# cszheng-ioa/Sixty-years-of-frequency-domain-monaural-speech-enhancement

Hardware: AMD Instinct MI355X
Metric: utterances/sec, 16 kHz 4 s clips, DCCRN decode (STFT->network->iSTFT) (higher is better)
Workload: dtype f32; 1 GPU; BASELINE configs[2]: DCCRN complex-mask, compressed input (0.5/2.0), 16 kHz x 4 s clips, batch 256 per MI355X, utterance-sharded; batch_per_gpu=256, global_batch=256, clip_samples=64000, parallelism=utterance shard x1 + RCCL gather to rank 0

## Files before the change

sixty-years-of-frequency-domain-monaural-speech-enhancement_amd/csrc/gemmconv.h:

```cpp
#pragma once
#include <hip/hip_runtime.h>
#include <vector>

namespace se {

constexpr int GC_MAX_TAPS = 16;
constexpr int GC_MAX_ROWS = 8;
constexpr int GC_MAX_KCP = 48;
constexpr int GC_TAB_KOFF = GC_MAX_ROWS + 2 * GC_MAX_TAPS;
constexpr int gc_kcp_max(int BM) { return 32; }
constexpr int gc_bld_max(int BM) { return (BM >= 128 || BM <= 32) ? 9 : 13; }
constexpr int gc_blocks_per_cu(int BM) { return BM <= 32 ? 6 : 3; }

enum Act : int { ACT_NONE = 0, ACT_PRELU = 1, ACT_ELU = 2, ACT_SOFTPLUS = 3, ACT_SIGMOID = 4, ACT_TANH = 5, ACT_RELU = 6 };
enum Epi : int {
    EPI_ACT = 0,
    EPI_LSTM = 1,
    EPI_GLU = 2,
    EPI_ADD = 3,
    EPI_MUL = 4,
    EPI_CMB = 5,
};

constexpr int GC_THIN_NT = 8;

struct GCParams {
    const float* A;
    const float* Ws;
    const float* bias;
    const float* slope;
    const float* post_scale;
    const float* post_shift;
    const float* bias_pad;
    int pad_lo;
    long ps_z;
    int cmb_neg;
    const float* cmb_i;
    float* cmb_s;
    const float* src0;
    const float* src1;
    float* dst;
    float* dst_elu;
    const float* aux;
    float* cell;
    long A_z, bias_z, src0_z, src1_z, dst_z, aux_z, cell_z;
    long s0_b, s0_c, s0_f;
    long s1_b, s1_c, s1_f;
    long d_b, d_c, d_f;
    long x_b, x_c, x_f;
    int C0, C1;
    int Fin, Tin;
    int B, Q, Tout, M, Mp;
    int si, so, po;
    int ntaps, nrows, dtmin, Wp;
    int CI_C, KC, KCp, nchunks;
    int act, epi;
    int n_ttiles, n_mtiles, Z;
    int dbg;
    int first_step;
    int gru;
    unsigned long long* timing;
    const unsigned* desc4;
    int t_base;
    int tb_soft;
    int pw4;
    int causal;
    const int* tlen;
    int qt2, qq_off, Qt;
    int pair, po2, fo_lim;
    short tdf[GC_MAX_TAPS], tdt[GC_MAX_TAPS];
    int nbuf;
    int trim;
    const unsigned* desc;
    const int* tab;
    float* stats;
    long st_b, st_c, st_f;
    float* cstats;
    long cs_b, cs_f;
    float* fz;
    long fz_b, fz_c, fz_f, fz_im;
    long fz_s;
    const float* nrm0;
    const float* nrm1;
    int flat_upr;
    int flat_units;
};
constexpr int GC_NRM_MAXC = 128;
constexpr int GC_FLAT_NRM_ROWS = 2;

struct GCGeom {
    int* tab = nullptr;
    unsigned* desc = nullptr;
    unsigned* desc4 = nullptr;
};
struct GCTail {
    int BN = 0, Wp = 0;
    GCGeom g;
};

struct GCSmallGeom {
    int dfmin = 0, dfmax = 0, dtmin = 0, dtmax = 0;
};

struct GCPlan {
    GCParams p{};
    int BM = 128, BN = 128;
    int lookback = 0;
    double flop_scale = 1.0;
    float* dA = nullptr;
    float* dWs = nullptr;
    unsigned* dDesc = nullptr;
    unsigned* dDesc4 = nullptr;
    GCSmallGeom small;
    bool tail_split = false;
    GCTail tail[3];
    GCTail qt2;
    GCTail flat[2];
    int flat_uw = 0;
    int qt2_nrows = 0, qt2_qoff = 0;
    float* dBias = nullptr;
    float* dSlope = nullptr;
    int* dTab = nullptr;
    float* dBiasPad = nullptr;
    float* dPostScale = nullptr;
    float* dPostShift = nullptr;
};

struct TapSpec {
    int ntaps = 0;
    int df[GC_MAX_TAPS];
    int dt[GC_MAX_TAPS];
};

GCPlan gc_make_plan(int M, int Cin, const TapSpec& taps, const std::vector<float>& w_logical,
                    const std::vector<float>& bias, const std::vector<float>& slope, int act, int epi,
                    int si, int so, int po, int tout_hint, int z = 1, int C0split = -1);
void gc_free_plan(GCPlan& pl);

void gc_register_overread_range(const void* lo, size_t bytes);
void gc_unregister_overread_range(const void* lo);

bool gc_stats_supported(const GCPlan& pl);
bool gc_nrm_supported(const GCPlan& pl);
void gc_launch(const GCPlan& pl, GCParams p, hipStream_t stream);
bool gc_launch_thin_pair(const GCParams& p0, const GCParams& p1, hipStream_t stream);

enum GCFamily : int { GC_FAM_TILE = 0, GC_FAM_THIN = 1, GC_FAM_THIN_PAIR = 2, GC_FAM_DIRECT = 3, GC_FAM_DIRECT_LDS = 4 };
struct GCLaunchRec {
    int family = GC_FAM_TILE;
    int BM = 0, BN = 0;
    int flat_upr = 0, upt = 0;
    int flat_rows = 0;
    int qt2 = 0, nrm = 0, res = 0, trim = 0, stats = 0, ragged = 0;
    int flat_nrm_refused = 0;
    long nblk = 0;
    int epi = 0, gru = 0;
};
void gc_set_launch_log(std::vector<GCLaunchRec>* log);
int gc_flat_rows_spanned(int B, int upr, int upt);

}
```

sixty-years-of-frequency-domain-monaural-speech-enhancement_amd/csrc/gemmconv.hip:

```cpp
#include "gemmconv.h"
#include "common.h"
#include "fastmath.h"
#include <algorithm>
#include <cmath>
#include <cstring>
#include <mutex>
#include <type_traits>

namespace se {

typedef float floatx16 __attribute__((ext_vector_type(16)));
typedef float floatx4 __attribute__((ext_vector_type(4)));

template <int N, typename F>
__device__ __forceinline__ void static_for(F&& f) {
    if constexpr (N > 0) {
        static_for<N - 1>(f);
        f(std::integral_constant<int, N - 1>{});
    }
}

__device__ __forceinline__ float fsig_(float x) { return fm_sigmoid(x); }
__device__ __forceinline__ float ftanh_(float x) { return fm_tanh(x); }
__device__ __forceinline__ float act_apply(float v, int act, float slope) {
    switch (act) {
        case ACT_PRELU: return v >= 0.f ? v : slope * v;
        case ACT_ELU: return v > 0.f ? v : fm_expm1(v);
        case ACT_SOFTPLUS: return fm_softplus(v);
        case ACT_SIGMOID: return fsig_(v);
        case ACT_TANH: return ftanh_(v);
        case ACT_RELU: return fmaxf(v, 0.f);
        default: return v;
    }
}
__device__ __forceinline__ float sigmoidf_(float v) { return 1.f / (1.f + expf(-v)); }
__device__ __forceinline__ float gc_fuse1(float v, float* __restrict__ zr, long im, long so = 0) {
    const float re = zr[0], ii = zr[im];
    const float cm = fm_sqrt(fmaxf(re * re + ii * ii, 1.1920928955078125e-07f));
    const float s = fsig_(v);
    zr[0] = re + s;
    zr[im] = ii + s;
    if (so) zr[so] = (re + s) + (ii + s);
    return v + fsig_(cm);
}

__device__ __forceinline__ void gc_dma16(const float* g, float* lds_wave_base) {
    const unsigned l = __builtin_amdgcn_readfirstlane((unsigned)(size_t)(__attribute__((address_space(3))) float*)lds_wave_base);
    asm volatile("s_mov_b32 m0, %0\n\ts_nop 0\n\tglobal_load_lds_dwordx4 %1, off" ::"s"(l), "v"(g) : "memory");
}
__device__ __forceinline__ void gc_dma4_masked(const float* g, unsigned lds_wave_base, unsigned pred) {
    unsigned long long saved;
    asm volatile(
        "s_mov_b64 %0, exec\n\t"
        "v_cmp_ne_u32_e32 vcc, 0, %1\n\t"
        "s_and_b64 exec, exec, vcc\n\t"
        "s_mov_b32 m0, %2\n\t"
        "s_nop 0\n\t"
        "global_load_lds_dword %3, off\n\t"
        "s_mov_b64 exec, %0"
        : "=&s"(saved)
        : "v"(pred), "s"(__builtin_amdgcn_readfirstlane(lds_wave_base)), "v"(g)
        : "memory", "vcc");
}
__device__ __forceinline__ void gc_dma16_masked(const float* g, unsigned lds_wave_base, unsigned pred) {
    unsigned long long saved;
    asm volatile(
        "s_mov_b64 %0, exec\n\t"
        "v_cmp_ne_u32_e32 vcc, 0, %1\n\t"
        "s_and_b64 exec, exec, vcc\n\t"
        "s_mov_b32 m0, %2\n\t"
        "s_nop 0\n\t"
        "global_load_lds_dwordx4 %3, off\n\t"
        "s_mov_b64 exec, %0"
        : "=&s"(saved)
        : "v"(pred), "s"(__builtin_amdgcn_readfirstlane(lds_wave_base)), "v"(g)
        : "memory", "vcc");
}
__device__ __forceinline__ void gc_dma16_s(const float* base, unsigned voff, unsigned lds_byte) {
    asm volatile("s_mov_b32 m0, %0\n\ts_nop 0\n\tglobal_load_lds_dwordx4 %1, %2" ::"s"(lds_byte), "v"(voff), "s"(base) : "memory");
}
__device__ __forceinline__ void gc_dma4_masked_s(const float* base, unsigned voff, unsigned lds_byte, unsigned vbits, unsigned mask) {
    unsigned long long saved;
    unsigned tmp;
    asm volatile(
        "s_mov_b64 %0, exec\n\t"
        "v_and_b32_e32 %1, %6, %2\n\t"
        "v_cmp_ne_u32_e32 vcc, 0, %1\n\t"
        "s_and_b64 exec, exec, vcc\n\t"
        "s_mov_b32 m0, %3\n\t"
        "s_nop 0\n\t"
        "global_load_lds_dword %4, %5\n\t"
        "s_mov_b64 exec, %0"
        : "=&s"(saved), "=&v"(tmp)
        : "v"(vbits), "s"(lds_byte), "v"(voff), "s"(base), "s"(mask)
        : "memory", "vcc");
}
__device__ __forceinline__ void gc_dma16_masked_s(const float* base, unsigned voff, unsigned lds_byte, unsigned vbits, unsigned mask) {
    unsigned long long saved;
    unsigned tmp;
    asm volatile(
        "s_mov_b64 %0, exec\n\t"
        "v_and_b32_e32 %1, %6, %2\n\t"
        "v_cmp_ne_u32_e32 vcc, 0, %1\n\t"
        "s_and_b64 exec, exec, vcc\n\t"
        "s_mov_b32 m0, %3\n\t"
        "s_nop 0\n\t"
        "global_load_lds_dwordx4 %4, %5\n\t"
        "s_mov_b64 exec, %0"
        : "=&s"(saved), "=&v"(tmp)
        : "v"(vbits), "s"(lds_byte), "v"(voff), "s"(base), "s"(mask)
        : "memory", "vcc");
}
__device__ __forceinline__ unsigned lds_addr(const float* p) {
    return (unsigned)(size_t)(__attribute__((address_space(3))) const float*)p;
}

#ifdef GC_TIMING
#define GC_T(SLOT)                                                               \
    {                                                                            \
        const unsigned long long now_ = __builtin_amdgcn_s_memtime();            \
        if (tid == 0) tacc[SLOT] += now_ - tlast;                                \
        tlast = __builtin_amdgcn_s_memtime();                                    \
    }
#else
#define GC_T(SLOT)
#endif

__device__ __forceinline__ float dpp_add8(float x) {
    x += __int_as_float(__builtin_amdgcn_update_dpp(0, __float_as_int(x), 0xB1, 0xF, 0xF, true));
    x += __int_as_float(__builtin_amdgcn_update_dpp(0, __float_as_int(x), 0x4E, 0xF, 0xF, true));
    x += __int_as_float(__builtin_amdgcn_update_dpp(0, __float_as_int(x), 0x141, 0xF, 0xF, true));
    return x;
}

template <int BM, int BN, int WM, int WN, int EPI, bool RES = false, bool TRIM = false, bool FZ = false, bool NRM = false, int FLATW = 0>
__global__ __launch_bounds__(256, RES ? 1 : (FZ || (BM >= 128 && BN >= 256)) ? (BM <= 32 ? 4 : 2) : gc_blocks_per_cu(BM)) void gc_kernel(const GCParams p) {
#ifdef GC_TIMING
    unsigned long long tacc[12] = {0, 0, 0, 0, 0, 0, 0, 0, 0, 0, 0, 0};
    unsigned long long tlast = __builtin_amdgcn_s_memtime();
#endif
    constexpr int TM = BM / (WM * 32);
    constexpr int TN = BN / (WN * 32);
    constexpr bool FLAT = FLATW > 0;
    constexpr int UW = FLAT ? FLATW : 32;
    constexpr int UPT = BN / 32;
    static_assert(!FLAT || (!RES && !TRIM && !FZ && EPI != EPI_LSTM), "flattened column tiles: plain offline variants only");
    constexpr int KCP_MAX = gc_kcp_max(BM);
    constexpr int A_IT = (KCP_MAX * BM / 4 + 255) / 256;
    constexpr int NB = BN >= 256 ? (BM >= 128 ? 6 : 5) : gc_bld_max(BM);
    static_assert(WM * WN == 4, "4 waves");

    extern __shared__ __attribute__((aligned(16))) float smem[];
    const int rows = p.CI_C * p.nrows;
    const int npatch = rows * p.Wp;
    const int bit = (npatch + 255) >> 8;
    const bool pw4 = p.pw4 != 0;
    constexpr bool fixt = TRIM;
    const int bit4 = (npatch / 4 + 255) >> 8;
    const int nA4 = p.KCp * (BM / 4);
    const int ait = (nA4 + 255) >> 8;
    const int As_sz = ait * 1024;
    const int Bs_sz = bit * 256;
    const int nbuf = RES ? p.nbuf : 2;
    float* As = smem;
    float* Bs = smem + nbuf * As_sz;

    const int tid = threadIdx.x;
    const int lane = tid & 63;
    const int wave = tid >> 6;
    const unsigned wave_u = __builtin_amdgcn_readfirstlane((unsigned)wave);
    const int l31 = lane & 31;
    const int hi = lane >> 5;

    int lid;
    {
        const int nblk = gridDim.x, id = blockIdx.x;
        const int xcd = id & 7, slot = id >> 3, q8 = nblk >> 3, r8 = nblk & 7;
        lid = (xcd < r8 ? xcd * (q8 + 1) : r8 * (q8 + 1) + (xcd - r8) * q8) + slot;
    }
    const int mt = lid % p.n_mtiles;
    int rest = lid / p.n_mtiles;
    const int ttile = FLAT ? (rest / p.Qt) % p.n_ttiles : rest % p.n_ttiles;
    if (FLAT) rest = (rest % p.Qt) + (rest / (p.Qt * p.n_ttiles)) * p.Qt;
    else rest /= p.n_ttiles;
    const bool qt2 = !FLAT && p.qt2 != 0;
    const int q = (rest % p.Qt) << (qt2 ? 1 : 0);
    rest /= p.Qt;
    const int u0 = FLAT ? ttile * UPT : 0;
    const int b = FLAT ? u0 / p.flat_upr : rest % p.B;
    const int z = FLAT ? rest : rest / p.B;
    const int t0 = FLAT ? p.t_base + (u0 - b * p.flat_upr) * 32 : p.t_base + ttile * (qt2 ? BN / 2 : BN);
    const int m0 = mt * BM;

    const float* __restrict__ Ag = p.A + (long)z * p.A_z + m0;

    constexpr int NPAIR = KCP_MAX / 2;
    constexpr bool KOFF_REGS = (BM >= 128 || TM * TN >= 4);
    int koffv[KOFF_REGS ? NPAIR : 1];
    constexpr int STRIPS = 4 * (TM * 32) * 36;
    int* tabl = reinterpret_cast<int*>(smem + max(nbuf * (As_sz + Bs_sz), STRIPS + (p.cstats ? 2048 : 0)));
    int* koff_lds = tabl + GC_TAB_KOFF;
    float* ep = reinterpret_cast<float*>(tabl + GC_TAB_KOFF + KCP_MAX + 8);
    constexpr int NRMB = FLAT ? GC_FLAT_NRM_ROWS : 1;
    static_assert(GC_FLAT_NRM_ROWS == 2, "the nrmC / nrmK fills below serve a tile's first row and the one after it");
    floatx4* nrmC = reinterpret_cast<floatx4*>(ep + 4 * BM);
    floatx4* nrmK = nrmC + NRMB * GC_NRM_MAXC;
    int* utab = reinterpret_cast<int*>(nrmC + (NRM ? NRMB * GC_NRM_MAXC + 2 * NRMB * KCP_MAX + 2 : 0));
    float* cpart = smem + STRIPS;
    GC_T(7);
    const int tabv = (tid < GC_TAB_KOFF + KCP_MAX + 8) ? p.tab[tid] : 0;
    const int fo = q * p.so + p.po;
    const float* __restrict__ bias = (fo < p.pad_lo) ? p.bias_pad : (p.bias ? p.bias + (long)z * p.bias_z : nullptr);
    float epv[4] = {0.f, 0.f, 1.f, 0.f};
    if (EPI != EPI_LSTM && tid < BM) {
        const int m = min(m0 + tid, p.M - 1);
        epv[0] = bias ? bias[m] : 0.f;
        const float lin_slope = p.act == ACT_NONE ? 1.f : 0.f;
        if (EPI == EPI_CMB) {
            epv[0] = p.post_shift[(long)z * p.ps_z + m];
            epv[1] = p.slope ? p.slope[(long)z * p.ps_z + m] : 1.f;
            epv[2] = p.post_scale[(long)z * p.ps_z + m];
        } else if (EPI != EPI_GLU) {
            epv[1] = (p.act == ACT_PRELU && p.slope) ? p.slope[m] : lin_slope;
        } else if (tid < BM / 2) {
            const int oc = min((m0 >> 1) + tid, (p.M >> 1) - 1);
            epv[1] = (p.act == ACT_PRELU && p.slope) ? p.slope[oc] : lin_slope;
            epv[2] = p.post_scale ? p.post_scale[oc] : 1.f;
            epv[3] = p.post_scale ? p.post_shift[oc] : 0.f;
        }
    }
    if constexpr (NRM) {
        const int ct_ = p.C0 + p.C1;
        if (tid < NRMB * ct_) {
            const int db_ = tid >= ct_ ? 1 : 0, ch_ = tid - db_ * ct_;
            const bool s1 = ch_ >= p.C0;
            const float* __restrict__ np_ = s1 ? p.nrm1 : p.nrm0;
            floatx4 v = {1.f, 0.f, 0.f, 0.f};
            if (np_) v = reinterpret_cast<const floatx4*>(np_)[(long)min(b + db_, p.B - 1) * (s1 ? p.C1 : p.C0) + (s1 ? ch_ - p.C0 : ch_)];
            nrmC[db_ * GC_NRM_MAXC + ch_] = v;
        }
    }
    if constexpr (FLAT) {
        if (tid < UPT) {
            const int u_ = u0 + tid, bk_ = u_ / p.flat_upr;
            utab[4 * tid + 0] = bk_ - b;
            utab[4 * tid + 1] = p.t_base + (u_ - bk_ * p.flat_upr) * 32;
            utab[4 * tid + 2] = u_ < p.flat_units ? 1 : 0;
            utab[4 * tid + 3] = p.tlen ? p.tlen[min(bk_, p.B - 1)] : 0x7fffffff;
        }
    }
    for (int i = tid; i < nbuf * Bs_sz / 4; i += 256) reinterpret_cast<floatx4*>(Bs)[i] = floatx4{0.f, 0.f, 0.f, 0.f};
    if (tid < GC_TAB_KOFF + KCP_MAX + 8) tabl[tid] = tabv;
    if (EPI != EPI_LSTM && tid < BM) {
        ep[tid] = epv[0];
        ep[BM + tid] = epv[1];
        if (EPI == EPI_GLU && tid < BM / 2) {
            ep[2 * BM + tid] = epv[2];
            ep[3 * BM + tid] = epv[3];
        }
        if (EPI == EPI_CMB) ep[2 * BM + tid] = epv[2];
    }
    __syncthreads();
    if constexpr (KOFF_REGS) {
        static_for<NPAIR>([&](auto KP) {
            constexpr int kp = decltype(KP)::value;
            koffv[kp] = koff_lds[2 * kp + hi];
        });
    }

    int nk_cil = 0, pb_cil = 0;
    bool nk_ok = false;
    const int npadL = (NRM && !FLAT) ? max(0, -(t0 + p.dtmin)) : 0;
    if constexpr (NRM) {
        if (tid < NRMB * KCP_MAX) {
            const int kr_ = tid & (KCP_MAX - 1);
            nk_cil = kr_ / p.ntaps;
            const int f = q * p.si + tabl[tabl[GC_MAX_ROWS + kr_ - nk_cil * p.ntaps]];
            nk_ok = kr_ < p.KC && f >= 0 && f < p.Fin;
        }
        pb_cil = tid / p.nrows;
    }

    unsigned aoff[A_IT];
    static_for<A_IT>([&](auto I) {
        constexpr int i = decltype(I)::value;
        int idx = tid + i * 256;
        if (idx >= nA4) idx = nA4 - 1;
        aoff[i] = 4u * (unsigned)((idx / (BM / 4)) * p.Mp + (idx % (BM / 4)) * 4);
    });
    unsigned boff[NB];
    unsigned vbits = 0;
    unsigned fullbits = 0;

    floatx16 acc[TM][TN];
#pragma unroll
    for (int i = 0; i < TM; ++i)
#pragma unroll
        for (int j = 0; j < TN; ++j)
#pragma unroll
            for (int r = 0; r < 16; ++r) acc[i][j][r] = 0.f;

    const int wm = wave / WN, wn = (WN == 4 && BN >= 256) ? ((wave + ttile) & 3) : wave % WN;
    constexpr int WNT = WN >= 2 ? WN / 2 : 1;
    const int wq = (qt2 && WN >= 2) ? wn / WNT : 0;
    const int wt = (qt2 && WN >= 2) ? wn % WNT : wn;
    const int am = wm * (TM * 32) + l31;
    const int bn = FLAT ? wn * (TN * UW) + l31 : wq * p.qq_off + wt * (TN * 32) + l31;
    const int jact = FLAT ? max(0, min(TN, p.flat_units - u0 - wn * TN))
                          : (q + wq >= p.Q) ? 0 : max(0, min(TN, (p.Tout - t0 - wt * (TN * 32) + 31) >> 5));

    int gchunk = 0;
    int buf = 0;

#define GC_MAKE_DESC(LIM)                                                                          \
    {                                                                                              \
        const int lim_ = (LIM);                                                                    \
        vbits = 0;                                                                                 \
         \
         \
         \
        unsigned dsc_[NB];                                                                         \
        {                                                                                          \
            const unsigned* __restrict__ dp_ = (pw4 ? p.desc4 : p.desc) + tid;                     \
            static_for<NB>([&](auto E) {                                                           \
                constexpr int e = decltype(E)::value;                                              \
                dsc_[e] = dp_[256 * e];                                                            \
            });                                                                                    \
        }                                                                                          \
        static_for<NB>([&](auto E) {                                                               \
            constexpr int e = decltype(E)::value;                                                  \
            const unsigned d_ = dsc_[e];                                                           \
            const int w = d_ & 0xfff, r = (d_ >> 12) & 0xf, cil = (d_ >> 16) & 0x7fff;             \
            const bool staged = (d_ >> 31) != 0;                                                   \
            const int f = q * p.si + tabl[staged ? r : 0];                                         \
             \
            const int uk_ = FLAT ? min(w / UW, UPT - 1) : 0;                                       \
            const int t = FLAT ? utab[4 * uk_ + 1] + p.dtmin + (w - uk_ * UW) : t0 + p.dtmin + w;  \
            const bool uok_ = !FLAT || utab[4 * uk_ + 2] != 0;                                     \
            const unsigned ub_ = (FLAT && uok_) ? (unsigned)utab[4 * uk_] * sb32 : 0u;             \
            const int fc = f < 0 ? 0 : (f >= p.Fin ? p.Fin - 1 : f);                               \
            const int tc = t < 0 ? 0 : (t >= p.Tin ? p.Tin - 1 : t);                               \
            const int cc = cil < lim_ ? cil : lim_ - 1;                                            \
            boff[e] = staged ? 4u * (ub_ + (unsigned)cc * sc32 + (unsigned)fc * sf32 + (unsigned)tc) : 0u;    \
             \
            vbits |= (staged && uok_ && (cil < lim_) && (f >= 0) && (f < p.Fin) && (t >= 0) && (t < p.Tin)) ? (1u << e) : 0u; \
             \
            if (fixt) vbits |= (staged && (t < p.Tin) && (t + 4 > p.Tin)) ? (0x10000u << e) : 0u;   \
        });                                                                                        \
         \
        fullbits = 0;       \
        {                                                                                          \
            if (!(p.dbg & 32)) static_for<NB>([&](auto E) {                                                           \
                constexpr int e = decltype(E)::value;                                              \
                if (e < bit4 && __builtin_amdgcn_ballot_w64((vbits >> e) & 1u) == ~0ull) fullbits |= 1u << e; \
            });                                                                                    \
        }                                                                                          \
    }
#define GC_TRIM_TAIL(BUF)                                                                          \
    if (fixt && (vbits >> 16)) {                                                                   \
        float* fb_ = Bs + (BUF) * Bs_sz + 4 * tid;                                                 \
        const int nv_ = p.Tin & 3;                                                                 \
        static_for<NB>([&](auto E) {                                                               \
            constexpr int e = decltype(E)::value;                                                  \
            if (vbits & (0x10000u << e)) {                                                         \
                _Pragma("unroll") for (int k = 1; k < 4; ++k)                                      \
                    if (k >= nv_) fb_[1024 * e + k] = 0.f;                                         \
            }                                                                                      \
        });                                                                                        \
    }
#define GC_LOAD_CHUNK(CH, BUF)                                                                     \
    {                                                                                              \
        if constexpr (NRM) {                                                                       \
             \
             \
            const int cb_ = (CH) * p.CI_C, co_ = seg ? p.C0 : 0;                                   \
            if (tid < NRMB * KCP_MAX) {                                                            \
                const int db_ = tid >= KCP_MAX ? 1 : 0;                                            \
                floatx4 v_ = nrmC[db_ * GC_NRM_MAXC + min(cb_ + nk_cil, Cseg - 1) + co_];          \
                if (!nk_ok) {                                                                      \
                    v_[0] = 0.f;                                                                   \
                    v_[1] = 0.f;                                                                   \
                }                                                                                  \
                nrmK[(BUF) * (NRMB * KCP_MAX) + tid] = v_;                                         \
            }                                                                                      \
            if (npadL > 0 && tid < rows) {                                                         \
                const float x0_ = nrmC[min(cb_ + pb_cil, Cseg - 1) + co_][3];                      \
                float* d_ = Bs + (BUF) * Bs_sz + tid * p.Wp;                                       \
                for (int w_ = 0; w_ < npadL; w_ += 4) *reinterpret_cast<floatx4*>(d_ + w_) = floatx4{x0_, x0_, x0_, x0_}; \
            }                                                                                      \
            if constexpr (FLAT) {       \
                if (tid < rows && p.dtmin < 0) {                                                   \
                    _Pragma("unroll") for (int k_ = 0; k_ < UPT; ++k_) {                           \
                        if (utab[4 * k_ + 1] + p.dtmin < 0 && utab[4 * k_ + 2]) {                  \
                            const float x0_ = nrmC[utab[4 * k_] * GC_NRM_MAXC + min(cb_ + pb_cil, Cseg - 1) + co_][3]; \
                            float* d_ = Bs + (BUF) * Bs_sz + tid * p.Wp + k_ * UW;                 \
                            for (int w_ = 0; w_ < -(utab[4 * k_ + 1] + p.dtmin); w_ += 4)          \
                                *reinterpret_cast<floatx4*>(d_ + w_) = floatx4{x0_, x0_, x0_, x0_}; \
                        }                                                                          \
                    }                                                                              \
                }                                                                                  \
            }                                                                                      \
        }                                                                                          \
         \
         \
        const float* __restrict__ Bc = sbase + (long)(CH) * p.CI_C * s_c;                          \
        const unsigned bb = __builtin_amdgcn_readfirstlane(lds_addr(Bs + (BUF) * Bs_sz));          \
        const unsigned bl = bb + 256u * wave_u, bl4 = bb + 1024u * wave_u;                         \
        if (pw4 && fullbits == (1u << bit4) - 1u) {      \
            static_for<NB>([&](auto E) {                                                           \
                constexpr int e = decltype(E)::value;                                              \
                if (e < bit4) gc_dma16_s(Bc, boff[e], bl4 + 4096u * e);                            \
            });                                                                                    \
        } else if (pw4) {                                                                          \
            static_for<NB>([&](auto E) {                                                           \
                constexpr int e = decltype(E)::value;                                              \
                if (e < bit4) gc_dma16_masked_s(Bc, boff[e], bl4 + 4096u * e, vbits, 1u << e);     \
            });                                                                                    \
        } else {                                                                                   \
            static_for<NB>([&](auto E) {                                                           \
                constexpr int e = decltype(E)::value;                                              \
                if (e < bit) gc_dma4_masked_s(Bc, boff[e], bl + 1024u * e, vbits, 1u << e);         \
            });                                                                                    \
        }                                                                                          \
        const float* __restrict__ Ac = Ag + (long)(gchunk + (CH)) * p.KCp * p.Mp;                  \
                                              \
        const unsigned Adw = __builtin_amdgcn_readfirstlane(lds_addr(As + (BUF) * As_sz)) + 1024u * wave_u; \
        static_for<A_IT>([&](auto I) {                                                             \
            constexpr int i = decltype(I)::value;                                                  \
            if (i < ait) gc_dma16_s(Ac, aoff[i], Adw + 4096u * i);                                 \
        });                                                                                        \
    }
#define GC_WAIT_CHUNK() asm volatile("s_waitcnt vmcnt(0)" ::: "memory")

    for (int seg = 0; seg < 2; ++seg) {
        const int Cseg = seg ? p.C1 : p.C0;
        if (Cseg <= 0) continue;
        const float* __restrict__ sbase =
            (seg ? p.src1 + (long)z * p.src1_z + (long)b * p.s1_b : p.src0 + (long)z * p.src0_z + (long)b * p.s0_b);
        const long s_c = seg ? p.s1_c : p.s0_c, s_f = seg ? p.s1_f : p.s0_f;
        const unsigned sc32 = (unsigned)s_c, sf32 = (unsigned)s_f;
        const unsigned sb32 = (unsigned)(seg ? p.s1_b : p.s0_b);
        const int nch = (Cseg + p.CI_C - 1) / p.CI_C;
        const int tail = Cseg - (nch - 1) * p.CI_C;

        GC_T(9);
        GC_MAKE_DESC(nch > 1 ? p.CI_C : tail);
        GC_T(10);
        if constexpr (RES) {
            buf = 0;
            for (int c2 = 0; c2 < min(nch, nbuf); ++c2) {
                if (c2 + 1 == nch && nch > 1 && tail != p.CI_C) GC_MAKE_DESC(tail);
                GC_LOAD_CHUNK(c2, c2);
            }
        } else {
            GC_LOAD_CHUNK(0, buf);
        }
        GC_T(1);
        GC_WAIT_CHUNK();
        GC_TRIM_TAIL(buf);
        GC_T(3);
        __syncthreads();
        GC_T(4);

        for (int c = 0; c < nch; ++c) {
            if constexpr (RES) {
                if (c > 0 && buf == nbuf) {
                    __syncthreads();
                    for (int c2 = c; c2 < min(nch, c + nbuf); ++c2) {
                        if (c2 + 1 == nch && tail != p.CI_C) GC_MAKE_DESC(tail);
                        GC_LOAD_CHUNK(c2, c2 - c);
                    }
                    GC_WAIT_CHUNK();
                    __syncthreads();
                    buf = 0;
                }
            }
            if (!RES && c + 1 < nch && !(p.dbg & 1)) {
                if (__builtin_expect(c + 2 == nch && tail != p.CI_C, 0)) GC_MAKE_DESC(tail);
                GC_LOAD_CHUNK(c + 1, buf ^ 1);
            }
            GC_T(1);
            const float* Ab = As + buf * As_sz + hi * BM + am;
            const float* Bb = Bs + buf * Bs_sz + bn;
            const floatx4* nkb = nrmK + buf * (NRMB * KCP_MAX) + hi;
            int nkd[FLAT && NRM ? TN : 1];
            if constexpr (FLAT && NRM) {
#pragma unroll
                for (int j = 0; j < TN; ++j) nkd[j] = utab[4 * min(wn * TN + j, UPT - 1)] * KCP_MAX;
            }
            const int npair = p.KCp >> 1;
#define GC_FETCH(KP, AR, BR)                                                                       \
    {                                                                                              \
        int o_;                                                                                    \
        if constexpr (KOFF_REGS) o_ = koffv[(KP) < NPAIR ? (KP) : NPAIR - 1];                      \
        else o_ = koff_lds[2 * (KP) + hi];                                                         \
        _Pragma("unroll") for (int i = 0; i < TM; ++i) AR[i] = Ab[(2 * (KP)) * BM + i * 32];       \
        _Pragma("unroll") for (int j = 0; j < JN; ++j) BR[j] = Bb[o_ + j * UW];                    \
        if constexpr (NRM && !FLAT) {                                                              \
            const floatx4 pr_ = nkb[2 * (KP)];                                                     \
            _Pragma("unroll") for (int j = 0; j < JN; ++j) {                                       \
                const float t_ = fmaf(BR[j], pr_[0], pr_[1]);                                      \
                BR[j] = fmaf(fminf(t_, 0.f), pr_[2], t_);                                          \
            }                                                                                      \
        }                                                                                          \
        if constexpr (NRM && FLAT) {                                                               \
            _Pragma("unroll") for (int j = 0; j < JN; ++j) {                                       \
                const floatx4 pr_ = nkb[2 * (KP) + nkd[j]];                                        \
                const float t_ = fmaf(BR[j], pr_[0], pr_[1]);                                      \
                BR[j] = fmaf(fminf(t_, 0.f), pr_[2], t_);                                          \
            }                                                                                      \
        }                                                                                          \
    }
#define GC_MMA(AR, BR)                                                                             \
    _Pragma("unroll") for (int i = 0; i < TM; ++i)                                                 \
        _Pragma("unroll") for (int j = 0; j < JN; ++j)                                             \
            acc[i][j] = __builtin_amdgcn_mfma_f32_32x32x2f32(AR[i], BR[j], acc[i][j], 0, 0, 0);
            auto mma_chunk = [&](auto JN_) {
                constexpr int JN = decltype(JN_)::value;
                float ax[TM], bx[JN], ay[TM], by[JN];
                GC_FETCH(0, ax, bx);
                static_for<NPAIR / 2>([&](auto KP2) {
                    constexpr int kp = 2 * decltype(KP2)::value;
                    int np_ = npair;
                    asm volatile("" : "+s"(np_));
                    if (kp < np_) {
                        constexpr int NDS = (TM + 1) / 2 + (JN + 1) / 2 + (NRM ? (FLAT ? JN : 1) : 0);
                        GC_FETCH(kp + 1, ay, by);
                        __builtin_amdgcn_sched_group_barrier(0x100, NDS, 0);
                        GC_MMA(ax, bx);
                        __builtin_amdgcn_sched_group_barrier(0x008, TM * JN, 0);
                        if constexpr (NRM) __builtin_amdgcn_sched_group_barrier(0x002, 3 * JN, 0);
                        GC_FETCH(kp + 2, ax, bx);
                        __builtin_amdgcn_sched_group_barrier(0x100, NDS, 0);
                        GC_MMA(ay, by);
                        __builtin_amdgcn_sched_group_barrier(0x008, TM * JN, 0);
                        if constexpr (NRM) __builtin_amdgcn_sched_group_barrier(0x002, 3 * JN, 0);
                    }
                });
            };
            if (!(p.dbg & 4)) {
                if (jact == 1 && TN == 2) mma_chunk(std::integral_constant<int, 1>{});
                else if (jact >= 1) mma_chunk(std::integral_constant<int, TN>{});
            }
#undef GC_FETCH
#undef GC_MMA
            GC_T(2);
            if constexpr (RES) {
                buf += 1;
            } else {
                GC_WAIT_CHUNK();
                GC_TRIM_TAIL(buf ^ 1);
                GC_T(3);
                __syncthreads();
                GC_T(4);
                buf ^= 1;
            }
        }
        if constexpr (RES) __syncthreads();
        gchunk += nch;
    }
#undef GC_MAKE_DESC
#undef GC_LOAD_CHUNK
#undef GC_WAIT_CHUNK
#undef GC_TRIM_TAIL

    if (p.dbg & 8) return;
    GC_T(0);
    const int fow = fo + wq * p.so;
    float* __restrict__ dst = p.dst + (long)z * p.dst_z + (long)b * p.d_b + (long)fow * p.d_f;

    constexpr int OROWS = (EPI == EPI_GLU) ? TM * 16 : TM * 32;
    constexpr bool GC_STATS = (EPI == EPI_GLU) || (EPI == EPI_ACT && BM == 64);
    constexpr int OST = 32 + 4;
    float* strip = smem + wave * (TM * 32 * OST);
#define GC_WAVE_FENCE() asm volatile("s_waitcnt lgkmcnt(0)" ::: "memory")
    if (EPI == EPI_ACT || EPI == EPI_ADD || EPI == EPI_MUL || EPI == EPI_GLU || EPI == EPI_CMB) {
        const int mw = wm * (TM * 32) + 4 * hi;
        const int lr = lane >> 3, lc = (lane & 7) * 4;
        const int mo0 = (EPI == EPI_GLU ? (m0 >> 1) : m0) + wm * OROWS;
        const int Mo = (q + wq < p.Q) ? ((EPI == EPI_GLU) ? (p.M >> 1) : p.M) : 0;
        const int tvalid0 = p.tlen ? p.tlen[b] : 0x7fffffff;
        const float* __restrict__ res =
            (EPI == EPI_ADD || EPI == EPI_MUL || EPI == EPI_CMB) ? p.aux + (long)z * p.aux_z + (long)b * p.x_b + (long)fow * p.x_f : nullptr;
        const float cmb_sg = (EPI == EPI_CMB && ((p.cmb_neg >> z) & 1)) ? -1.f : 1.f;
        const float* __restrict__ cmbi = (EPI == EPI_CMB && p.cmb_s) ? p.cmb_i + (long)b * p.d_b + (long)fow * p.d_f : nullptr;
        float* __restrict__ cmbs = (EPI == EPI_CMB && p.cmb_s) ? p.cmb_s + (long)b * p.d_b + (long)fow * p.d_f : nullptr;
        float* __restrict__ delu = (EPI == EPI_GLU && p.dst_elu) ? p.dst_elu + (long)b * p.d_b + (long)fow * p.d_f : nullptr;
        float* __restrict__ fzb = FZ ? p.fz + (long)b * p.fz_b + (long)fow * p.fz_f : nullptr;
        auto epi_tile = [&](auto jc) __attribute__((always_inline)) {
            constexpr int j = decltype(jc)::value;
            if (j > 0) GC_WAVE_FENCE();
            const int uk = FLAT ? min(wn * TN + j, UPT - 1) : 0;
            const long dbJ = FLAT ? utab[4 * uk] : 0;
            const int tj0 = FLAT ? utab[4 * uk + 1] : t0 + wt * (TN * 32) + j * 32;
            const int MoJ = (!FLAT || utab[4 * uk + 2]) ? Mo : 0;
            const int tvalid = FLAT ? utab[4 * uk + 3] : tvalid0;
            const int tstat = min(p.Tout, tvalid);
            float* __restrict__ dstJ = dst + dbJ * p.d_b;
            const float* __restrict__ resJ = res ? res + dbJ * p.x_b : nullptr;
            const float* __restrict__ cmbiJ = cmbi ? cmbi + dbJ * p.d_b : nullptr;
            float* __restrict__ cmbsJ = cmbs ? cmbs + dbJ * p.d_b : nullptr;
            float* __restrict__ deluJ = delu ? delu + dbJ * p.d_b : nullptr;
            constexpr bool PRE = (EPI == EPI_ADD || EPI == EPI_MUL || EPI == EPI_CMB);
            const int tgp = tj0 + lc;
            floatx4 rvp[PRE ? OROWS / 8 : 1], zre[FZ ? OROWS / 8 : 1], zim[FZ ? OROWS / 8 : 1], ivp[EPI == EPI_CMB ? OROWS / 8 : 1];
            if ((PRE || FZ) && tgp + 3 < p.Tout && MoJ > 0) {
#pragma unroll
                for (int it = 0; it < OROWS / 8; ++it) {
                    const int m = min(mo0 + it * 8 + lr, MoJ - 1);
                    if (PRE) rvp[it] = *reinterpret_cast<const floatx4*>(resJ + (long)m * p.x_c + tgp);
                    if (EPI == EPI_CMB && cmbiJ) ivp[it] = *reinterpret_cast<const floatx4*>(cmbiJ + (long)m * p.d_c + tgp);
                    if (FZ) {
                        zre[it] = *reinterpret_cast<const floatx4*>(fzb + (long)m * p.fz_c + tgp);
                        zim[it] = *reinterpret_cast<const floatx4*>(fzb + (long)m * p.fz_c + tgp + p.fz_im);
                    }
                }
            }
            auto write_strip = [&](auto ACT_) __attribute__((always_inline)) {
                constexpr int ACT = decltype(ACT_)::value;
                auto actf = [&](float v, float sl) __attribute__((always_inline)) -> float {
                    if constexpr (ACT == -2) return v;
                    else if constexpr (ACT < 0) return v >= 0.f ? v : sl * v;
                    else return act_apply(v, ACT, sl);
                };
                typedef float floatx2 __attribute__((ext_vector_type(2)));
#pragma unroll
                for (int i = 0; i < TM; ++i) {
                    if (EPI == EPI_CMB) {
#pragma unroll
                        for (int r = 0; r < 16; ++r) {
                            const int dm = i * 32 + (r & 3) + 8 * (r >> 2);
                            strip[(4 * hi + dm) * OST + l31] = acc[i][j][r];
                        }
                    } else if (EPI != EPI_GLU) {
#pragma unroll
                        for (int g4 = 0; g4 < 4; ++g4) {
                            const int dm0 = i * 32 + 8 * g4;
                            const floatx4 b4 = *reinterpret_cast<const floatx4*>(ep + mw + dm0);
                            floatx4 s4 = {1.f, 1.f, 1.f, 1.f};
                            if constexpr (ACT != -2) s4 = *reinterpret_cast<const floatx4*>(ep + BM + mw + dm0);
#pragma unroll
                            for (int k = 0; k < 4; ++k) {
                                const float v = acc[i][j][4 * g4 + k] + b4[k];
                                strip[(4 * hi + dm0 + k) * OST + l31] = actf(v, s4[k]);
                            }
                        }
                    } else {
#pragma unroll
                        for (int g4 = 0; g4 < 4; ++g4) {
                            const int dm0 = i * 32 + 8 * g4;
                            const int ol0 = (mw + dm0) >> 1;
                            const floatx4 b4 = *reinterpret_cast<const floatx4*>(ep + mw + dm0);
                            const floatx2 sc2 = *reinterpret_cast<const floatx2*>(ep + 2 * BM + ol0);
                            const floatx2 sh2 = *reinterpret_cast<const floatx2*>(ep + 3 * BM + ol0);
                            floatx2 sl2 = {1.f, 1.f};
                            if constexpr (ACT != -2) sl2 = *reinterpret_cast<const floatx2*>(ep + BM + ol0);
#pragma unroll
                            for (int k = 0; k < 2; ++k) {
                                const float a = acc[i][j][4 * g4 + 2 * k] + b4[2 * k];
                                const float g = acc[i][j][4 * g4 + 2 * k + 1] + b4[2 * k + 1];
                                float v = a * fsig_(g);
                                v = v * sc2[k] + sh2[k];
                                strip[(((4 * hi + dm0) >> 1) + k) * OST + l31] = actf(v, sl2[k]);
                            }
                        }
                    }
                }
            };
            switch (p.act) {
                case ACT_NONE: write_strip(std::integral_constant<int, -2>{}); break;
                case ACT_RELU:
                case ACT_PRELU: write_strip(std::integral_constant<int, -1>{}); break;
                case ACT_ELU: write_strip(std::integral_constant<int, ACT_ELU>{}); break;
                case ACT_SOFTPLUS: write_strip(std::integral_constant<int, ACT_SOFTPLUS>{}); break;
                case ACT_SIGMOID: write_strip(std::integral_constant<int, ACT_SIGMOID>{}); break;
                default: write_strip(std::integral_constant<int, ACT_TANH>{}); break;
            }
            GC_WAVE_FENCE();
            const int tg = tj0 + lc;
            constexpr int RB_UNROLL = (PRE || FZ) ? OROWS / 8 : 1;
            float ccs[GC_STATS ? 4 : 1] = {}, ccq[GC_STATS ? 4 : 1] = {};
            long doff = (long)(mo0 + lr) * p.d_c + tg;
            const long dstep = 8L * p.d_c;
            long soff = 0;
            if constexpr (GC_STATS) soff = (long)(b + dbJ) * p.st_b + (long)(mo0 + lr) * p.st_c + (long)fow * p.st_f + (tj0 >> 5) * 2;
            const long sstep = GC_STATS ? 8L * p.st_c : 0;
#pragma unroll RB_UNROLL
            for (int it = 0; it < OROWS / 8; ++it, doff += dstep, soff += sstep) {
                const int row = it * 8 + lr, m = mo0 + row;
                floatx4 v = *reinterpret_cast<const floatx4*>(strip + row * OST + lc);
                if constexpr (GC_STATS) {
                    if (p.cstats && m < MoJ) {
#pragma unroll
                        for (int k = 0; k < 4; ++k) {
                            const float xk = (tg + k < tstat) ? v[k] : 0.f;
                            ccs[k] += xk;
                            ccq[k] = fmaf(xk, xk, ccq[k]);
                        }
                    }
                }
                if constexpr (GC_STATS) {
                    if (p.stats) {
                        float s = 0.f, q = 0.f;
#pragma unroll
                        for (int k = 0; k < 4; ++k) {
                            const float xk = (tg + k < tstat) ? v[k] : 0.f;
                            s += xk;
                            q = fmaf(xk, xk, q);
                        }
                        s = dpp_add8(s);
                        q = dpp_add8(q);
                        const int tb = tg - lc;
                        if ((lane & 7) == 0 && m < MoJ && tb < p.Tout) {
                            float* sp = p.stats + soff;
                            sp[0] = s;
                            sp[1] = q;
                        }
                    }
                }
                if (m < MoJ) {
                    float* __restrict__ dp = dstJ + doff;
                    if (__builtin_expect(tg + 3 < p.Tout, 1)) {
                        if (EPI == EPI_ADD || EPI == EPI_MUL) v = (EPI == EPI_ADD) ? v + rvp[it] : v * rvp[it];
                        if (EPI == EPI_CMB) {
                            const int rt = wm * (TM * 32) + row;
                            const float sh_ = ep[rt], sl_ = ep[BM + rt], sc_ = ep[2 * BM + rt];
#pragma unroll
                            for (int k = 0; k < 4; ++k) {
                                const float u = fmaf(fmaf(cmb_sg, v[k], rvp[it][k]), sc_, sh_);
                                v[k] = u >= 0.f ? u : sl_ * u;
                            }
                        }
                        if (__builtin_expect(tg + 3 >= tvalid, 0)) {
#pragma unroll
                            for (int k = 0; k < 4; ++k) v[k] = (tg + k < tvalid) ? v[k] : 0.f;
                        }
                        if (FZ) {
                            float* __restrict__ zr = fzb + (long)m * p.fz_c + tg;
                            floatx4 re = zre[it], ii = zim[it];
#pragma unroll
                            for (int k = 0; k < 4; ++k) {
                                const float cm = fm_sqrt(fmaxf(re[k] * re[k] + ii[k] * ii[k], 1.1920928955078125e-07f));
                                const float sg = fsig_(v[k]);
                                re[k] += sg;
                                ii[k] += sg;
                                v[k] += fsig_(cm);
                            }
                            *reinterpret_cast<floatx4*>(zr) = re;
                            *reinterpret_cast<floatx4*>(zr + p.fz_im) = ii;
                            if (p.fz_s) *reinterpret_cast<floatx4*>(zr + p.fz_s) = re + ii;
                        }
                        *reinterpret_cast<floatx4*>(dp) = v;
                        if (EPI == EPI_GLU && deluJ) {
                            floatx4 e4;
#pragma unroll
                            for (int k = 0; k < 4; ++k) e4[k] = v[k] > 0.f ? v[k] : fm_expm1(v[k]);
                            *reinterpret_cast<floatx4*>(deluJ + doff) = e4;
                        }
                        if (EPI == EPI_CMB && cmbsJ) {
                            floatx4 s4 = v + ivp[it];
                            if (__builtin_expect(tg + 3 >= tvalid, 0)) {
#pragma unroll
                                for (int k = 0; k < 4; ++k) s4[k] = (tg + k < tvalid) ? s4[k] : 0.f;
                            }
                            *reinterpret_cast<floatx4*>(cmbsJ + doff) = s4;
                        }
                    } else {
#pragma unroll
                        for (int k = 0; k < 4; ++k)
                            if (tg + k < p.Tout) {
                                float o = v[k];
                                if (EPI == EPI_ADD) o += resJ[(long)m * p.x_c + tg + k];
                                if (EPI == EPI_MUL) o *= resJ[(long)m * p.x_c + tg + k];
                                if (EPI == EPI_CMB) {
                                    const int rt = wm * (TM * 32) + row;
                                    const float u = fmaf(fmaf(cmb_sg, o, resJ[(long)m * p.x_c + tg + k]), ep[2 * BM + rt], ep[rt]);
                                    o = u >= 0.f ? u : ep[BM + rt] * u;
                                }
                                o = (tg + k < tvalid) ? o : 0.f;
                                if (FZ) o = gc_fuse1(o, fzb + (long)m * p.fz_c + tg + k, p.fz_im, p.fz_s);
                                dp[k] = o;
                                if (EPI == EPI_GLU && deluJ) deluJ[doff + k] = o > 0.f ? o : fm_expm1(o);
                                if (EPI == EPI_CMB && cmbsJ) {
                                    const float iv = cmbiJ[doff + k];
                                    cmbsJ[doff + k] = (tg + k < tvalid) ? o + iv : 0.f;
                                }
                            }
                    }
                }
            }
            if constexpr (GC_STATS) {
                if (p.cstats) {
#pragma unroll
                    for (int k = 0; k < 4; ++k) {
                        ccs[k] += __int_as_float(__builtin_amdgcn_update_dpp(0, __float_as_int(ccs[k]), 0x128, 0xF, 0xF, true));
                        ccq[k] += __int_as_float(__builtin_amdgcn_update_dpp(0, __float_as_int(ccq[k]), 0x128, 0xF, 0xF, true));
                    }
                    if (!(lane & 8)) {
                        float* cp_ = cpart + (((wm * 4 + (lane >> 4)) * BN) + wt * (TN * 32) + j * 32 + lc) * 2;
#pragma unroll
                        for (int k = 0; k < 4; ++k) {
                            cp_[2 * k] = ccs[k];
                            cp_[2 * k + 1] = ccq[k];
                        }
                    }
                }
            }
        };
        epi_tile(std::integral_constant<int, 0>{});
        if constexpr (TN > 1) epi_tile(std::integral_constant<int, 1>{});
        if constexpr (TN > 2) {
            epi_tile(std::integral_constant<int, 2>{});
            epi_tile(std::integral_constant<int, 3>{});
        }
        static_assert(TN == 1 || TN == 2 || TN == 4, "epilogue: column tiles per wave");
        if constexpr (GC_STATS) {
            if (p.cstats) {
                __syncthreads();
                for (int col = tid; col < BN; col += 256) {
                    float a = 0.f, c2 = 0.f;
#pragma unroll
                    for (int w = 0; w < 4 * WM; ++w) {
                        a += cpart[(w * BN + col) * 2];
                        c2 += cpart[(w * BN + col) * 2 + 1];
                    }
                    const int ukc = FLAT ? col >> 5 : 0;
                    const int t = FLAT ? utab[4 * ukc + 1] + (col & 31) : t0 + col;
                    const long bc = FLAT ? b + utab[4 * ukc] : b;
                    if (t < p.Tout && fo < p.so * p.Q + p.po && (!FLAT || utab[4 * ukc + 2])) {
                        float* cg = p.cstats + bc * p.cs_b + (long)fo * p.cs_f + 2 * t;
                        cg[0] = a;
                        cg[1] = c2;
                    }
                }
            }
        }
    } else {
        const bool has_gx = p.aux != nullptr;
        const float* __restrict__ gx = has_gx ? p.aux + (long)z * p.aux_z + (long)b * p.x_b + (long)fo * p.x_f : p.bias;
        float* __restrict__ cell = p.cell + (long)z * p.cell_z + (long)b * p.d_b + (long)fo * p.d_f;
        float cpa[TM][TN][4];
#pragma unroll
        for (int i = 0; i < TM; ++i)
#pragma unroll
            for (int j = 0; j < TN; ++j) {
                const int tc = min(t0 + wn * (TN * 32) + j * 32 + l31, p.Tout - 1);
                const int mb = m0 + wm * (TM * 32) + i * 32 + 4 * hi;
#pragma unroll
                for (int g4 = 0; g4 < 4; ++g4) {
                    const int m = min(mb + 8 * g4, p.M - 4);
                    cpa[i][j][g4] = p.first_step ? 0.f : cell[(long)(m >> 2) * p.d_c + tc];
                }
            }
        auto cells = [&](auto GRU_, auto HGX_) __attribute__((always_inline)) {
            constexpr bool GRU = decltype(GRU_)::value, HGX = decltype(HGX_)::value;
#pragma unroll
        for (int i = 0; i < TM; ++i)
#pragma unroll
            for (int j = 0; j < TN; ++j) {
                const int t = t0 + wn * (TN * 32) + j * 32 + l31;
                const int tc = min(t, p.Tout - 1);
                const int mb = m0 + wm * (TM * 32) + i * 32 + 4 * hi;
                float g[16], cp[4];
#pragma unroll
                for (int g4 = 0; g4 < 4; ++g4) {
                    const int m = min(mb + 8 * g4, p.M - 4);
                    const float* gp = HGX ? gx + (long)m * p.x_c + tc : gx + m;
                    const long gs = HGX ? p.x_c : 1;
#pragma unroll
                    for (int k = 0; k < 4; ++k) g[4 * g4 + k] = gp[(long)k * gs];
                    cp[g4] = cpa[i][j][g4];
                }
#pragma unroll
                for (int g4 = 0; g4 < 4; ++g4) {
                    const int m = mb + 8 * g4;
                    const float gi = acc[i][j][4 * g4 + 0] + g[4 * g4 + 0];
                    const float gf = acc[i][j][4 * g4 + 1] + g[4 * g4 + 1];
                    const float gg = acc[i][j][4 * g4 + 2] + g[4 * g4 + 2];
                    const float go = acc[i][j][4 * g4 + 3] + g[4 * g4 + 3];
                    float cn, hn;
                    if constexpr (GRU) {
                        const float r = fsig_(gi), zz = fsig_(gf);
                        const float hw = acc[i][j][4 * g4 + 2] + go;
                        const float nn = ftanh_(g[4 * g4 + 2] + r * hw);
                        hn = (1.f - zz) * nn + zz * cp[g4];
                        cn = hn;
                    } else {
                        cn = fsig_(gf) * cp[g4] + fsig_(gi) * ftanh_(gg);
                        hn = fsig_(go) * ftanh_(cn);
                    }
                    if (m + 3 < p.M && t < p.Tout) {
                        const long oi = (long)(m >> 2) * p.d_c + t;
                        cell[oi] = cn;
                        dst[oi] = hn;
                    }
                }
            }
    
        };
        if (p.gru) {
            if (has_gx) cells(std::true_type{}, std::true_type{});
            else cells(std::true_type{}, std::false_type{});
        } else {
            if (has_gx) cells(std::false_type{}, std::true_type{});
            else cells(std::false_type{}, std::false_type{});
        }
    }
#ifdef GC_TIMING
    GC_T(5);
    if (tid == 0) {
        for (int i = 0; i < 6; ++i) atomicAdd(p.timing + i, tacc[i]);
        for (int i = 7; i < 12; ++i) atomicAdd(p.timing + i, tacc[i]);
        atomicAdd(p.timing + 6, 1ull);
    }
#endif
}

template <int MM, int EPI>
__global__ __launch_bounds__(256) void gc_small_kernel(const GCParams p) {
    __shared__ int s_df[GC_MAX_TAPS], s_dt[GC_MAX_TAPS];
    if (threadIdx.x < p.ntaps) {
        s_df[threadIdx.x] = p.tab[p.tab[GC_MAX_ROWS + threadIdx.x]];
        s_dt[threadIdx.x] = p.tab[GC_MAX_ROWS + GC_MAX_TAPS + threadIdx.x];
    }
    __syncthreads();
    int lid;
    {
        const int nblk = gridDim.x, id = blockIdx.x;
        const int xcd = id & 7, slot = id >> 3, q8 = nblk >> 3, r8 = nblk & 7;
        lid = (xcd < r8 ? xcd * (q8 + 1) : r8 * (q8 + 1) + (xcd - r8) * q8) + slot;
    }
    const int q = lid % p.Q;
    int rest = lid / p.Q;
    const int nt = (p.Tout + 255) >> 8;
    const int tt = rest % nt;
    rest /= nt;
    const int b = rest % p.B, z = rest / p.B;
    const int t = tt * 256 + threadIdx.x;
    const int tc = min(t, p.Tout - 1);
    float acc[MM];
#pragma unroll
    for (int m = 0; m < MM; ++m) acc[m] = 0.f;
    const float* __restrict__ W = p.Ws + (long)z * (p.C0 + p.C1) * p.ntaps * MM;
#pragma unroll 1
    for (int seg = 0; seg < 2; ++seg) {
        const int C = seg ? p.C1 : p.C0;
        if (C == 0) continue;
        const float* __restrict__ src = seg ? p.src1 + (long)z * p.src1_z + (long)b * p.s1_b
                                            : p.src0 + (long)z * p.src0_z + (long)b * p.s0_b;
        const long s_c = seg ? p.s1_c : p.s0_c, s_f = seg ? p.s1_f : p.s0_f;
        const float* __restrict__ Wc = W + (long)(seg ? p.C0 : 0) * p.ntaps * MM;
        for (int j = 0; j < p.ntaps; ++j) {
            const int fi = q * p.si + s_df[j], ti = tc + s_dt[j];
            const bool ok = fi >= 0 && fi < p.Fin && ti >= 0 && ti < p.Tin;
            const float* __restrict__ xp = src + (long)min(max(fi, 0), p.Fin - 1) * s_f + min(max(ti, 0), p.Tin - 1);
            const float keep = ok ? 1.f : 0.f;
#pragma unroll 8
            for (int c = 0; c < C; ++c) {
                const float x = xp[(long)c * s_c] * keep;
                const float* __restrict__ w = Wc + ((long)c * p.ntaps + j) * MM;
#pragma unroll
                for (int m = 0; m < MM; ++m) acc[m] = fmaf(w[m], x, acc[m]);
            }
        }
    }
    if (t >= p.Tout) return;
    const int fo = q * p.so + p.po;
    const float* __restrict__ bias = (fo < p.pad_lo) ? p.bias_pad : (p.bias ? p.bias + (long)z * p.bias_z : nullptr);
    float* __restrict__ dst = p.dst + (long)z * p.dst_z + (long)b * p.d_b + (long)fo * p.d_f;
    const float* __restrict__ res = (EPI == EPI_ADD || EPI == EPI_MUL) ? p.aux + (long)z * p.aux_z + (long)b * p.x_b + (long)fo * p.x_f : nullptr;
    if constexpr (EPI == EPI_GLU) {
#pragma unroll
        for (int j = 0; j < MM / 2; ++j) {
            if (2 * j + 1 < p.M) {
                const float a = acc[2 * j] + (bias ? bias[2 * j] : 0.f), g = acc[2 * j + 1] + (bias ? bias[2 * j + 1] : 0.f);
                float v = a * fsig_(g);
                if (p.post_scale) v = v * p.post_scale[j] + p.post_shift[j];
                v = act_apply(v, p.act, p.slope ? p.slope[j] : 0.f);
                if (p.pair) {
                    const int cls = (2 * j) / p.pair, fo2 = q * p.so + (cls ? p.po2 : p.po);
                    if (fo2 < p.fo_lim) dst[(long)(fo2 - fo) * p.d_f + (long)(j - cls * (p.pair >> 1)) * p.d_c + t] = v;
                } else {
                    dst[(long)j * p.d_c + t] = v;
                }
            }
        }
        return;
    }
#pragma unroll
    for (int m = 0; m < MM; ++m) {
        if (m < p.M) {
            float v = acc[m] + (bias ? bias[m] : 0.f);
            v = act_apply(v, p.act, p.slope ? p.slope[m] : 0.f);
            if (EPI == EPI_ADD) v += res[(long)m * p.x_c + t];
            if (EPI == EPI_MUL) v *= res[(long)m * p.x_c + t];
            if (EPI == EPI_ACT && p.pair) {
                const int cls = m / p.pair, fo2 = q * p.so + (cls ? p.po2 : p.po);
                if (fo2 < p.fo_lim) dst[(long)(fo2 - fo) * p.d_f + (long)(m - cls * p.pair) * p.d_c + t] = v;
                continue;
            }
            dst[(long)m * p.d_c + t] = v;
        }
    }
}

constexpr int SQB = 8;
constexpr int SWT = 264;
template <int MM, int EPI, int SI>
__global__ __launch_bounds__(256) void gc_small_lds_kernel(const GCParams p, const int CC, const int NR, const int dfmin,
                                                           const int dtlo) {
    extern __shared__ float patch[];
    __shared__ int s_off[GC_MAX_TAPS];
    __shared__ float s_w[8 * GC_MAX_TAPS * MM];
    const int tid = threadIdx.x, lane = tid & 63, wave = tid >> 6;
    if (tid < p.ntaps)
        s_off[tid] = (p.tab[p.tab[GC_MAX_ROWS + tid]] - dfmin) * SWT + (p.tab[GC_MAX_ROWS + GC_MAX_TAPS + tid] - dtlo);
    const int QG = (p.Q + SQB - 1) / SQB;
    int rest = blockIdx.x;
    const int q0 = (rest % QG) * SQB;
    rest /= QG;
    const int nt = (p.Tout + 255) >> 8;
    const int tt = rest % nt;
    rest /= nt;
    const int b = rest % p.B, z = rest / p.B;
    const int t = tt * 256 + tid;
    const int f0 = q0 * SI + dfmin, tb = tt * 256 + dtlo;
    float acc[SQB][MM];
#pragma unroll
    for (int qq = 0; qq < SQB; ++qq)
#pragma unroll
        for (int m = 0; m < MM; ++m) acc[qq][m] = 0.f;
    const float* __restrict__ W = p.Ws + (long)z * (p.C0 + p.C1) * p.ntaps * MM;
    const int plane = NR * SWT;
#pragma unroll 1
    for (int seg = 0; seg < 2; ++seg) {
        const int C = seg ? p.C1 : p.C0;
        if (C == 0) continue;
        const float* __restrict__ src = seg ? p.src1 + (long)z * p.src1_z + (long)b * p.s1_b
                                            : p.src0 + (long)z * p.src0_z + (long)b * p.s0_b;
        const long s_c = seg ? p.s1_c : p.s0_c, s_f = seg ? p.s1_f : p.s0_f;
        const float* __restrict__ Wc = W + (long)(seg ? p.C0 : 0) * p.ntaps * MM;
        constexpr int SRB = 6, SWN = (SWT + 63) / 64, SWW = (8 * GC_MAX_TAPS * MM + 255) / 256;
        float sv[SRB][SWN], wv[SWW];
        auto issue = [&](int c0n) {
            const int ccn = min(CC, C - c0n);
#pragma unroll
            for (int i = 0; i < SRB; ++i) {
                const int row = min(wave + 4 * i, ccn * NR - 1);
                const int c = row / NR, r = row - c * NR;
                const float* __restrict__ sp = src + (long)(c0n + c) * s_c + (long)min(max(f0 + r, 0), p.Fin - 1) * s_f;
#pragma unroll
                for (int k = 0; k < SWN; ++k) sv[i][k] = sp[min(max(tb + lane + 64 * k, 0), p.Tin - 1)];
            }
#pragma unroll
            for (int k = 0; k < SWW; ++k) wv[k] = Wc[(long)c0n * p.ntaps * MM + min(tid + 256 * k, ccn * p.ntaps * MM - 1)];
        };
        issue(0);
#pragma unroll 1
        for (int c0 = 0; c0 < C; c0 += CC) {
            const int cc = min(CC, C - c0);
            __syncthreads();
#pragma unroll
            for (int k = 0; k < SWW; ++k)
                if (tid + 256 * k < cc * p.ntaps * MM) s_w[tid + 256 * k] = wv[k];
#pragma unroll
            for (int i = 0; i < SRB; ++i) {
                const int row = wave + 4 * i;
                if (row < cc * NR) {
                    const int c = row / NR, r = row - c * NR;
                    const int fi = f0 + r;
                    const bool rok = fi >= 0 && fi < p.Fin;
                    float* __restrict__ dp = patch + c * plane + r * SWT;
#pragma unroll
                    for (int k = 0; k < SWN; ++k) {
                        const int w = lane + 64 * k, ti = tb + w;
                        if (w < SWT) dp[w] = (rok && ti >= 0 && ti < p.Tin) ? sv[i][k] : 0.f;
                    }
                }
            }
            if (c0 + CC < C) issue(c0 + CC);
            __syncthreads();
            for (int c = 0; c < cc; ++c) {
                const float* __restrict__ pc = patch + c * plane + tid;
                const float* wc = s_w + c * p.ntaps * MM;
#pragma unroll 2
                for (int j = 0; j < p.ntaps; ++j) {
                    const float* __restrict__ pj = pc + s_off[j];
                    float w[MM];
#pragma unroll
                    for (int m = 0; m < MM; ++m) w[m] = wc[j * MM + m];
#pragma unroll
                    for (int qq = 0; qq < SQB; ++qq) {
                        const float x = pj[qq * SI * SWT];
#pragma unroll
                        for (int m = 0; m < MM; ++m) acc[qq][m] = fmaf(w[m], x, acc[qq][m]);
                    }
                }
            }
        }
    }
    if (t >= p.Tout) return;
#pragma unroll
    for (int qq = 0; qq < SQB; ++qq) {
        if (q0 + qq >= p.Q) break;
        const int fo = (q0 + qq) * p.so + p.po;
        const float* __restrict__ bias = (fo < p.pad_lo) ? p.bias_pad : (p.bias ? p.bias + (long)z * p.bias_z : nullptr);
        float* __restrict__ dst = p.dst + (long)z * p.dst_z + (long)b * p.d_b + (long)fo * p.d_f;
        const float* __restrict__ res = (EPI == EPI_ADD || EPI == EPI_MUL) ? p.aux + (long)z * p.aux_z + (long)b * p.x_b + (long)fo * p.x_f : nullptr;
        if constexpr (EPI == EPI_GLU) {
#pragma unroll
            for (int j = 0; j < MM / 2; ++j) {
                if (2 * j + 1 < p.M) {
                    const float a = acc[qq][2 * j] + (bias ? bias[2 * j] : 0.f), g = acc[qq][2 * j + 1] + (bias ? bias[2 * j + 1] : 0.f);
                    float v = a * fsig_(g);
                    if (p.post_scale) v = v * p.post_scale[j] + p.post_shift[j];
                    v = act_apply(v, p.act, p.slope ? p.slope[j] : 0.f);
                    if (p.pair) {
                        const int cls = (2 * j) / p.pair, fo2 = (q0 + qq) * p.so + (cls ? p.po2 : p.po);
                        if (fo2 < p.fo_lim) dst[(long)(fo2 - fo) * p.d_f + (long)(j - cls * (p.pair >> 1)) * p.d_c + t] = v;
                    } else {
                        dst[(long)j * p.d_c + t] = v;
                    }
                }
            }
            continue;
        }
#pragma unroll
        for (int m = 0; m < MM; ++m) {
            if (m < p.M) {
                float v = acc[qq][m] + (bias ? bias[m] : 0.f);
                v = act_apply(v, p.act, p.slope ? p.slope[m] : 0.f);
                if (EPI == EPI_ADD) v += res[(long)m * p.x_c + t];
                if (EPI == EPI_MUL) v *= res[(long)m * p.x_c + t];
                if (EPI == EPI_ACT && p.pair) {
                    const int cls = m / p.pair, fo2 = (q0 + qq) * p.so + (cls ? p.po2 : p.po);
                    if (fo2 < p.fo_lim) dst[(long)(fo2 - fo) * p.d_f + (long)(m - cls * p.pair) * p.d_c + t] = v;
                    continue;
                }
                dst[(long)m * p.d_c + t] = v;
            }
        }
    }
}

template <int EPI, int NT>
__device__ __forceinline__ void gc_thin_body(const GCParams& p, const int blk) {
    constexpr int RB = 8, KG = 32, UN = 8;
    __shared__ float part[KG][RB][NT + 1];
    __shared__ int s_df[GC_MAX_TAPS], s_dt[GC_MAX_TAPS];
    const int tid = threadIdx.x, mi = tid & (RB - 1), kg = tid / RB;
#pragma unroll
    for (int j = 0; j < GC_MAX_TAPS; ++j)
        if (tid == j) {
            s_df[j] = p.tdf[j];
            s_dt[j] = p.tdt[j];
        }
    __syncthreads();
    const int nm = (p.M + RB - 1) / RB;
    const int mt = blk % nm;
    const int rest = blk / nm;
    const int q = rest % p.Q, b = rest / p.Q;
    const int m = mt * RB + mi, t0 = p.t_base, n = p.Tout - p.t_base;
    const int ntaps = p.ntaps, Ktot = (p.C0 + p.C1) * ntaps;
    const int nch0 = p.C0 > 0 ? (p.C0 + p.CI_C - 1) / p.CI_C : 0;
    float acc[NT];
#pragma unroll
    for (int t = 0; t < NT; ++t) acc[t] = 0.f;
    for (int k0 = kg; k0 < Ktot; k0 += KG * UN) {
        float w[UN], xv[UN][NT];
#pragma unroll
        for (int u = 0; u < UN; ++u) {
            const int kk = k0 + u * KG;
            const bool kok = kk < Ktot;
            const int kc = kok ? kk : 0;
            const int ci = kc / ntaps, j = kc - ci * ntaps;
            const bool seg = ci >= p.C0;
            const int cs = seg ? ci - p.C0 : ci;
            const int chunk = (seg ? nch0 : 0) + cs / p.CI_C, cil = cs % p.CI_C;
            const float wv = p.A[((long)chunk * p.KCp + cil * ntaps + j) * p.Mp + m];
            const int f = q * p.si + s_df[j];
            const bool fok = kok && f >= 0 && f < p.Fin;
            const int fc = fok ? f : 0;
            const float* __restrict__ src = seg ? p.src1 + (long)b * p.s1_b + (long)cs * p.s1_c + (long)fc * p.s1_f
                                                : p.src0 + (long)b * p.s0_b + (long)cs * p.s0_c + (long)fc * p.s0_f;
            const int tb = t0 + s_dt[j];
            w[u] = fok ? wv : 0.f;
#pragma unroll
            for (int t = 0; t < NT; ++t) {
                const int ti = tb + t;
                const bool ok = t < n && ti >= 0 && ti < p.Tin;
                const float x = src[ok ? ti : 0];
                xv[u][t] = ok ? x : 0.f;
            }
        }
#pragma unroll
        for (int u = 0; u < UN; ++u)
#pragma unroll
            for (int t = 0; t < NT; ++t) acc[t] = fmaf(w[u], xv[u][t], acc[t]);
    }
#pragma unroll
    for (int t = 0; t < NT; ++t) part[kg][mi][t] = acc[t];
    __syncthreads();
    const bool fold = tid < RB * NT;
    const int r = tid & (RB - 1), t = (tid / RB) & (NT - 1);
    float tot = 0.f;
    if (fold) {
#pragma unroll
        for (int g = 0; g < KG; ++g) tot += part[g][r][t];
    }
    __syncthreads();
    if (fold) part[0][r][t] = tot;
    __syncthreads();
    if (!fold || t >= n) return;
    const int fo = q * p.so + p.po, mr = mt * RB + r;
    const float* __restrict__ bias = (fo < p.pad_lo) ? p.bias_pad : p.bias;
    float* __restrict__ dst = p.dst + (long)b * p.d_b + (long)fo * p.d_f + t0 + t;
    if (EPI == EPI_LSTM) {
        if ((r & 3) || mr + 3 >= p.M) return;
        const int tc = t0 + t;
        const bool has_gx = p.aux != nullptr;
        const float* __restrict__ gx = has_gx ? p.aux + (long)b * p.x_b + (long)fo * p.x_f + (long)mr * p.x_c + tc : p.bias + mr;
        const long gs = has_gx ? p.x_c : 1;
        float* __restrict__ cell = p.cell + (long)b * p.d_b + (long)fo * p.d_f + (long)(mr >> 2) * p.d_c + tc;
        const float g0 = gx[0], g1 = gx[gs], g2 = gx[2 * gs], g3 = gx[3 * gs];
        const float cp = p.first_step ? 0.f : *cell;
        const float gi = part[0][r][t] + g0, gf = part[0][r + 1][t] + g1, gg = part[0][r + 2][t] + g2, go = part[0][r + 3][t] + g3;
        float cn, hn;
        if (p.gru) {
            const float rr = fsig_(gi), zz = fsig_(gf);
            const float hw = part[0][r + 2][t] + go;
            const float nn = ftanh_(g2 + rr * hw);
            hn = (1.f - zz) * nn + zz * cp;
            cn = hn;
        } else {
            cn = fsig_(gf) * cp + fsig_(gi) * ftanh_(gg);
            hn = fsig_(go) * ftanh_(cn);
        }
        *cell = cn;
        dst[(long)(mr >> 2) * p.d_c] = hn;
    } else if (EPI == EPI_GLU) {
        if ((r & 1) || mr + 1 >= p.M) return;
        const int oc = mr >> 1;
        const float a = part[0][r][t] + (bias ? bias[mr] : 0.f), g = part[0][r + 1][t] + (bias ? bias[mr + 1] : 0.f);
        float v = a * fsig_(g);
        if (p.post_scale) v = v * p.post_scale[oc] + p.post_shift[oc];
        dst[(long)oc * p.d_c] = act_apply(v, p.act, p.slope ? p.slope[oc] : 0.f);
    } else {
        if (mr >= p.M) return;
        float v = part[0][r][t] + (bias ? bias[mr] : 0.f);
        v = act_apply(v, p.act, p.slope ? p.slope[mr] : 0.f);
        if (EPI == EPI_ADD || EPI == EPI_MUL) {
            const float rv = p.aux[(long)b * p.x_b + (long)fo * p.x_f + (long)mr * p.x_c + t0 + t];
            v = (EPI == EPI_ADD) ? v + rv : v * rv;
        }
        dst[(long)mr * p.d_c] = v;
    }
}
template <int EPI, int NT>
__global__ __launch_bounds__(256) void gc_thin_kernel(const GCParams p) {
    gc_thin_body<EPI, NT>(p, (int)blockIdx.x);
}
struct GCThinPair {
    GCParams p[2];
    int nblk0;
};
template <int EPI, int NT>
__global__ __launch_bounds__(256) void gc_thin_pair_kernel(const GCThinPair a) {
    const int cls = (int)blockIdx.x >= a.nblk0 ? 1 : 0;
    gc_thin_body<EPI, NT>(a.p[cls], (int)blockIdx.x - (cls ? a.nblk0 : 0));
}
template <int EPI>
static void gc_thin_launch_n(const GCParams& p, dim3 grid, int n, hipStream_t stream) {
    if (n <= 1) hipLaunchKernelGGL((gc_thin_kernel<EPI, 1>), grid, dim3(256), 0, stream, p);
    else if (n <= 2) hipLaunchKernelGGL((gc_thin_kernel<EPI, 2>), grid, dim3(256), 0, stream, p);
    else if (n <= 4) hipLaunchKernelGGL((gc_thin_kernel<EPI, 4>), grid, dim3(256), 0, stream, p);
    else hipLaunchKernelGGL((gc_thin_kernel<EPI, 8>), grid, dim3(256), 0, stream, p);
}
static thread_local std::vector<GCLaunchRec>* g_launch_log = nullptr;
static thread_local int g_flat_nrm_refused = 0;
void gc_set_launch_log(std::vector<GCLaunchRec>* log) { g_launch_log = log; }
static void gc_log_launch(int family, const GCParams& p, long nblk, int BM = 0, int BN = 0, bool res = false) {
    if (!g_launch_log) return;
    GCLaunchRec r;
    r.family = family;
    r.BM = BM;
    r.BN = BN;
    r.flat_upr = p.flat_upr;
    r.upt = p.flat_upr ? BN / 32 : 0;
    r.flat_rows = p.flat_upr ? gc_flat_rows_spanned(p.B, p.flat_upr, BN / 32) : 0;
    r.qt2 = p.qt2;
    r.nrm = (p.nrm0 || p.nrm1) ? 1 : 0;
    r.res = res ? 1 : 0;
    r.trim = p.trim;
    r.stats = (p.stats || p.cstats) ? 1 : 0;
    r.ragged = p.tlen ? 1 : 0;
    r.flat_nrm_refused = g_flat_nrm_refused;
    r.nblk = nblk;
    r.epi = p.epi;
    r.gru = p.gru;
    g_launch_log->push_back(r);
}
int gc_flat_rows_spanned(int B, int upr, int upt) {
    const long units = (long)B * upr, tiles = (units + upt - 1) / upt;
    int most = 0;
    for (long k = 0; k < std::min<long>(tiles, upr); ++k) {
        const long u0 = k * upt, u1 = std::min(u0 + upt, units) - 1;
        most = std::max(most, (int)(u1 / upr - u0 / upr + 1));
    }
    return most;
}

constexpr long GC_THIN_MAX_BLOCKS = 8192;
static long gc_thin_blocks(const GCParams& p) {
    const int n = p.Tout - p.t_base;
    if ((p.Ws && p.pair) || n > GC_THIN_NT || p.Z > 1 || p.stats || p.cstats || p.nrm0 || p.nrm1) return 0;
    if (p.epi != EPI_ACT && p.epi != EPI_ADD && p.epi != EPI_MUL && p.epi != EPI_GLU && p.epi != EPI_LSTM) return 0;
    if (p.epi == EPI_LSTM && (p.M & 3)) return 0;
    const long nblk = (long)((p.M + 7) >> 3) * p.Q * p.B;
    if (nblk > GC_THIN_MAX_BLOCKS) return 0;
    if (!p.Ws) {
        const int nt = n <= 1 ? 1 : (n <= 2 ? 2 : (n <= 4 ? 4 : 8));
        const double waves_thin = std::ceil((double)nblk / 2048.0);
        const double waves_mfma = std::ceil((double)std::max(p.Z, 1) * p.B * p.Q * std::max(p.n_mtiles, 1) / 512.0);
        if ((long)p.B * n > 64 || nblk > 2800 * waves_mfma || waves_thin * (1 + nt) > 12 * waves_mfma) return 0;
    }
    return nblk;
}
static bool gc_thin_launch(const GCParams& p, hipStream_t stream) {
    const long nblk = (p.fz || p.dst_elu) ? 0 : gc_thin_blocks(p);
    if (nblk <= 0) return false;
    const int n = p.Tout - p.t_base;
    dim3 grid((unsigned)nblk);
    switch (p.epi) {
        case EPI_ACT: gc_thin_launch_n<EPI_ACT>(p, grid, n, stream); break;
        case EPI_ADD: gc_thin_launch_n<EPI_ADD>(p, grid, n, stream); break;
        case EPI_MUL: gc_thin_launch_n<EPI_MUL>(p, grid, n, stream); break;
        case EPI_GLU: gc_thin_launch_n<EPI_GLU>(p, grid, n, stream); break;
        case EPI_LSTM: gc_thin_launch_n<EPI_LSTM>(p, grid, n, stream); break;
        default: return false;
    }
    SE_HIP(hipGetLastError());
    gc_log_launch(GC_FAM_THIN, p, nblk);
    return true;
}

template <int EPI>
static void gc_thin_pair_launch_n(const GCThinPair& a, dim3 grid, int n, hipStream_t stream) {
    if (n <= 1) hipLaunchKernelGGL((gc_thin_pair_kernel<EPI, 1>), grid, dim3(256), 0, stream, a);
    else if (n <= 2) hipLaunchKernelGGL((gc_thin_pair_kernel<EPI, 2>), grid, dim3(256), 0, stream, a);
    else if (n <= 4) hipLaunchKernelGGL((gc_thin_pair_kernel<EPI, 4>), grid, dim3(256), 0, stream, a);
    else hipLaunchKernelGGL((gc_thin_pair_kernel<EPI, 8>), grid, dim3(256), 0, stream, a);
}
bool gc_launch_thin_pair(const GCParams& p0, const GCParams& p1, hipStream_t stream) {
    const long n0 = gc_thin_blocks(p0), n1 = gc_thin_blocks(p1);
    if (n0 <= 0 || n1 <= 0 || p0.epi != p1.epi || p0.Tout - p0.t_base != p1.Tout - p1.t_base) return false;
    GCThinPair a;
    a.p[0] = p0;
    a.p[1] = p1;
    a.nblk0 = (int)n0;
    const int n = p0.Tout - p0.t_base;
    dim3 grid((unsigned)(n0 + n1));
    switch (p0.epi) {
        case EPI_ACT: gc_thin_pair_launch_n<EPI_ACT>(a, grid, n, stream); break;
        case EPI_ADD: gc_thin_pair_launch_n<EPI_ADD>(a, grid, n, stream); break;
        case EPI_MUL: gc_thin_pair_launch_n<EPI_MUL>(a, grid, n, stream); break;
        case EPI_GLU: gc_thin_pair_launch_n<EPI_GLU>(a, grid, n, stream); break;
        default: return false;
    }
    SE_HIP(hipGetLastError());
    gc_log_launch(GC_FAM_THIN_PAIR, p0, n0 + n1);
    return true;
}

template <int MM, int EPI>
static void gc_small_lds_launch(const GCParams& p, dim3 grid, size_t shm, int CC, int NR, const GCSmallGeom& sg, hipStream_t stream) {
    if (p.si == 1) hipLaunchKernelGGL((gc_small_lds_kernel<MM, EPI, 1>), grid, dim3(256), shm, stream, p, CC, NR, sg.dfmin, sg.dtmin);
    else hipLaunchKernelGGL((gc_small_lds_kernel<MM, EPI, 2>), grid, dim3(256), shm, stream, p, CC, NR, sg.dfmin, sg.dtmin);
}

template <int MM>
static void gc_small_launch(const GCParams& p, const GCSmallGeom& sg, hipStream_t stream) {
    const int NR = (SQB - 1) * p.si + (sg.dfmax - sg.dfmin) + 1;
    constexpr int small_kb = 24;
    const int CC = std::min(std::min(8, 24 / std::max(NR, 1)), (int)((size_t)small_kb * 1024 / ((size_t)NR * SWT * sizeof(float))));
    const long nblk8 = (long)((p.Tout + 255) / 256) * ((p.Q + SQB - 1) / SQB) * p.B * p.Z;
    if (CC >= 2 && p.Q >= SQB && (p.si == 1 || p.si == 2) && sg.dtmax - sg.dtmin <= SWT - 256 && nblk8 >= 4 * 256 &&
        (sg.dfmax - sg.dfmin >= 2 || (sg.dfmax - sg.dfmin >= 1 && MM >= 2 && p.C0 + p.C1 >= 64))) {
        SE_CHECK(nblk8 < (1L << 31), "grid size");
        const size_t shm = (size_t)CC * NR * SWT * sizeof(float);
        dim3 grid((unsigned)nblk8);
        switch (p.epi) {
            case EPI_ACT: gc_small_lds_launch<MM, EPI_ACT>(p, grid, shm, CC, NR, sg, stream); break;
            case EPI_ADD: gc_small_lds_launch<MM, EPI_ADD>(p, grid, shm, CC, NR, sg, stream); break;
            case EPI_MUL: gc_small_lds_launch<MM, EPI_MUL>(p, grid, shm, CC, NR, sg, stream); break;
            case EPI_GLU:
                if constexpr (MM >= 2) gc_small_lds_launch<MM, EPI_GLU>(p, grid, shm, CC, NR, sg, stream);
                break;
            default: SE_CHECK(false, "direct small-M path: unsupported epilogue");
        }
        SE_HIP(hipGetLastError());
        gc_log_launch(GC_FAM_DIRECT_LDS, p, nblk8);
        return;
    }
    const long nblk = (long)((p.Tout + 255) / 256) * p.Q * p.B * p.Z;
    SE_CHECK(nblk > 0 && nblk < (1L << 31), "grid size");
    dim3 grid((unsigned)nblk);
    switch (p.epi) {
        case EPI_ACT: hipLaunchKernelGGL((gc_small_kernel<MM, EPI_ACT>), grid, dim3(256), 0, stream, p); break;
        case EPI_ADD: hipLaunchKernelGGL((gc_small_kernel<MM, EPI_ADD>), grid, dim3(256), 0, stream, p); break;
        case EPI_MUL: hipLaunchKernelGGL((gc_small_kernel<MM, EPI_MUL>), grid, dim3(256), 0, stream, p); break;
        case EPI_GLU:
            if constexpr (MM >= 2) hipLaunchKernelGGL((gc_small_kernel<MM, EPI_GLU>), grid, dim3(256), 0, stream, p);
            break;
        default: SE_CHECK(false, "direct small-M path: unsupported epilogue");
    }
    SE_HIP(hipGetLastError());
    gc_log_launch(GC_FAM_DIRECT, p, nblk);
}

static size_t gc_lds_bytes(const GCParams& p, int BM, size_t epi_bytes, int nbuf = 2) {
    const size_t as = (size_t)((p.KCp * (BM / 4) + 255) / 256) * 1024, bs = (size_t)((p.CI_C * p.nrows * p.Wp + 255) / 256) * 256;
    const size_t nrb = p.flat_upr ? GC_FLAT_NRM_ROWS : 1;
    const size_t nrm = ((p.nrm0 || p.nrm1) ? (size_t)(nrb * GC_NRM_MAXC + 2 * nrb * gc_kcp_max(BM) + 2) * 16 : 0) + (p.flat_upr ? 128 : 0);
    const size_t cst = p.cstats ? (size_t)4 * 256 * 2 * 4 : 0;
    return std::max((size_t)nbuf * (as + bs) * 4, epi_bytes + cst) + (GC_TAB_KOFF + GC_MAX_KCP + 8) * 4 + (size_t)4 * BM * 4 + 64 + nrm;
}

GCGeom gc_build_geom(const TapSpec& taps, const std::vector<int>& rows, int dtmin, int nrows, int Wp, int cic, int KC, int NB) {
    GCGeom g;
    std::vector<int> tab(GC_TAB_KOFF + GC_MAX_KCP + 8, 0);
    for (int r = 0; r < nrows; ++r) tab[r] = rows[r];
    for (int j = 0; j < taps.ntaps; ++j) {
        tab[GC_MAX_ROWS + j] = (int)(std::find(rows.begin(), rows.end(), taps.df[j]) - rows.begin());
        tab[GC_MAX_ROWS + GC_MAX_TAPS + j] = taps.dt[j];
    }
    for (int k = 0; k < KC; ++k) {
        const int cil = k / taps.ntaps, j = k - cil * taps.ntaps;
        tab[GC_TAB_KOFF + k] = cil * (nrows * Wp) + tab[GC_MAX_ROWS + j] * Wp + (taps.dt[j] - dtmin);
    }
    SE_HIP(hipMalloc(&g.tab, tab.size() * sizeof(int)));
    SE_HIP(hipMemcpy(g.tab, tab.data(), tab.size() * sizeof(int), hipMemcpyHostToDevice));
    const int npatch = cic * nrows * Wp, gpr = Wp / 4;
    SE_CHECK(Wp % 4 == 0 && Wp < 4096 && nrows <= 16 && cic < 32768, "patch descriptor field overflow");
    std::vector<unsigned> desc((size_t)NB * 256, 0u), d4((size_t)NB * 256, 0u);
    for (int e = 0; e < NB; ++e)
        for (int t = 0; t < 256; ++t) {
            const int fe = t + 256 * e;
            if (fe < npatch) {
                const int rr = fe / Wp, w = fe - rr * Wp, cil = rr / nrows, r = rr - cil * nrows;
                desc[(size_t)e * 256 + t] = (unsigned)w | ((unsigned)r << 12) | ((unsigned)cil << 16) | 0x80000000u;
            }
            if (4 * fe < npatch) {
                const int rr = fe / gpr, w = 4 * (fe - rr * gpr), cil = rr / nrows, r = rr - cil * nrows;
                d4[(size_t)e * 256 + t] = (unsigned)w | ((unsigned)r << 12) | ((unsigned)cil << 16) | 0x80000000u;
            }
        }
    SE_HIP(hipMalloc(&g.desc, desc.size() * sizeof(unsigned)));
    SE_HIP(hipMemcpy(g.desc, desc.data(), desc.size() * sizeof(unsigned), hipMemcpyHostToDevice));
    SE_HIP(hipMalloc(&g.desc4, d4.size() * sizeof(unsigned)));
    SE_HIP(hipMemcpy(g.desc4, d4.data(), d4.size() * sizeof(unsigned), hipMemcpyHostToDevice));
    return g;
}

GCPlan gc_make_plan(int M, int Cin, const TapSpec& taps, const std::vector<float>& w, const std::vector<float>& bias,
                    const std::vector<float>& slope, int act, int epi, int si, int so, int po, int tout_hint, int Z,
                    int C0split) {
    const int C0 = (C0split < 0 || C0split > Cin) ? Cin : C0split;
    SE_CHECK(taps.ntaps >= 1 && taps.ntaps <= GC_MAX_TAPS, "tap count");
    SE_CHECK((long)w.size() == (long)Z * M * Cin * taps.ntaps, "weight size mismatch in gc_make_plan");
    GCPlan pl;
    GCParams& p = pl.p;
    pl.BM = M >= 96 ? 128 : (M >= 48 ? 64 : 32);
    {
        static const int pw64 = getenv("SE_GC_PW_BM64") ? atoi(getenv("SE_GC_PW_BM64")) : 128;
        if (pw64 > 0 && taps.ntaps == 1 && Cin <= pw64 && M >= 96 && M <= 384 && epi != EPI_LSTM) pl.BM = 64;
    }
    pl.BN = (tout_hint >= 96 || pl.BM == 32) ? 128 : 64;
    int dtmin = taps.dt[0], dtmax = taps.dt[0];
    std::vector<int> rows;
    for (int j = 0; j < taps.ntaps; ++j) {
        dtmin = std::min(dtmin, taps.dt[j]);
        dtmax = std::max(dtmax, taps.dt[j]);
        if (std::find(rows.begin(), rows.end(), taps.df[j]) == rows.end()) rows.push_back(taps.df[j]);
    }
    std::sort(rows.begin(), rows.end());
    SE_CHECK((int)rows.size() <= GC_MAX_ROWS, "too many distinct frequency rows");
    p.ntaps = taps.ntaps;
    p.nrows = (int)rows.size();
    for (int j = 0; j < taps.ntaps; ++j) {
        SE_CHECK(taps.df[j] >= -32768 && taps.df[j] <= 32767 && taps.dt[j] >= -32768 && taps.dt[j] <= 32767, "tap offset range");
        p.tdf[j] = (short)taps.df[j];
        p.tdt[j] = (short)taps.dt[j];
    }
    p.causal = dtmax <= 0;
    pl.lookback = std::max(-dtmin, 0);
    dtmin = -((std::max(-dtmin, 0) + 3) & ~3);
    dtmax = (std::max(dtmax, 0) + 3) & ~3;
    p.dtmin = dtmin;
    p.Wp = pl.BN + (dtmax - dtmin);
    SE_CHECK(p.nrows * p.Wp <= gc_bld_max(pl.BM) * 256, "tap span too wide for one staged patch");
    int cic = 1;
    double best = -1.0;
    for (int c = 1; c <= std::max(std::max(C0, Cin - C0), 1); ++c) {
        const int kc = c * taps.ntaps, kcp = (kc + 3) & ~3;
        const bool pw = taps.ntaps == 1;
        const int kmax = pw ? (pl.BM >= 128 ? 24 : 32) : gc_kcp_max(pl.BM);
        const int cap = gc_bld_max(pl.BM) * 256 * (pw ? 4 : 1);
        if (kcp > kmax || c * p.nrows * p.Wp > cap) continue;
        if (pl.BM == 64 && pl.BN == 128 && taps.ntaps > 1 && epi != EPI_LSTM && kc > 12 &&
            (long)c * p.nrows * (256 + (dtmax - dtmin)) > 4608)
            continue;
        const double score = (double)kc / kcp + 1e-4 * kc;
        if (score > best) {
            best = score;
            cic = c;
        }
    }
    p.CI_C = cic;
    p.KC = cic * taps.ntaps;
    p.KCp = (p.KC + 3) & ~3;
    SE_CHECK(p.KCp <= gc_kcp_max(pl.BM), "single-channel chunk exceeds K budget");
    {
        GCGeom g = gc_build_geom(taps, rows, dtmin, p.nrows, p.Wp, cic, p.KC, gc_bld_max(pl.BM));
        pl.dTab = g.tab;
        pl.dDesc = g.desc;
        pl.dDesc4 = g.desc4;
        p.tab = g.tab;
        p.desc = g.desc;
        p.desc4 = g.desc4;
        pl.tail_split = taps.ntaps != 1;
        if (pl.BN == 128 && pl.BM == 128) {
            pl.tail[0].BN = 32;
            pl.tail[0].Wp = 32 + (dtmax - dtmin);
            pl.tail[0].g = gc_build_geom(taps, rows, dtmin, p.nrows, pl.tail[0].Wp, cic, p.KC, gc_bld_max(pl.BM));
        }
        if (pl.BN == 128 && epi != EPI_LSTM && taps.ntaps > 1) {
            std::vector<int> r2 = rows;
            for (int r : rows)
                if (std::find(r2.begin(), r2.end(), r + si) == r2.end()) r2.push_back(r + si);
            std::sort(r2.begin(), r2.end());
            const bool interval = r2.back() - r2.front() + 1 == (int)r2.size();
            const int wp2 = 64 + (dtmax - dtmin);
            if (interval && (int)r2.size() <= GC_MAX_ROWS && (int)r2.size() < 2 * p.nrows &&
                cic * (int)r2.size() * wp2 <= gc_bld_max(pl.BM) * 256) {
                pl.qt2.BN = 64;
                pl.qt2.Wp = wp2;
                pl.qt2.g = gc_build_geom(taps, r2, dtmin, (int)r2.size(), wp2, cic, p.KC, gc_bld_max(pl.BM));
                pl.qt2_nrows = (int)r2.size();
                pl.qt2_qoff = si * wp2;
            }
        }
        if (pl.BN == 128 && pl.BM == 64 && epi != EPI_LSTM && taps.ntaps > 1) {
            pl.tail[2].BN = 256;
            pl.tail[2].Wp = 256 + (dtmax - dtmin);
            pl.tail[2].g = gc_build_geom(taps, rows, dtmin, p.nrows, pl.tail[2].Wp, cic, p.KC, gc_bld_max(pl.BM));
        }
        static const int wide128_env = getenv("SE_GC_WIDE128") ? atoi(getenv("SE_GC_WIDE128")) : 1;
        if (wide128_env && pl.BN == 128 && pl.BM == 128 && taps.ntaps == 1 && epi == EPI_LSTM && cic * 256 <= 6 * 1024) {
            pl.tail[2].BN = 256;
            pl.tail[2].Wp = 256;
            pl.tail[2].g = gc_build_geom(taps, rows, dtmin, p.nrows, 256, cic, p.KC, gc_bld_max(pl.BM));
        }
        static const int flat_env = getenv("SE_GC_FLAT") ? atoi(getenv("SE_GC_FLAT")) : 1;
        if (flat_env && pl.BM == 64 && pl.BN == 128 && epi != EPI_LSTM && p.causal && dtmin >= -4 && Z == 1) {
            const int uw = 32 - dtmin;
            pl.flat_uw = uw;
            const int nbk = gc_bld_max(pl.BM);
            if ((long)cic * p.nrows * 4 * uw <= (long)nbk * 256 * 4) {
                pl.flat[0].BN = 128;
                pl.flat[0].Wp = 4 * uw;
                pl.flat[0].g = gc_build_geom(taps, rows, dtmin, p.nrows, 4 * uw, cic, p.KC, nbk);
            }
            if (pl.BM == 64 && (long)cic * p.nrows * 8 * uw <= 4608) {
                pl.flat[1].BN = 256;
                pl.flat[1].Wp = 8 * uw;
                pl.flat[1].g = gc_build_geom(taps, rows, dtmin, p.nrows, 8 * uw, cic, p.KC, nbk);
            }
        }
        if (pl.BN == 128 && (pl.BM == 64 || pl.BM == 128) && epi != EPI_LSTM) {
            pl.tail[1].BN = 64;
            pl.tail[1].Wp = 64 + (dtmax - dtmin);
            pl.tail[1].g = gc_build_geom(taps, rows, dtmin, p.nrows, pl.tail[1].Wp, cic, p.KC, gc_bld_max(pl.BM));
        }
    }
    const int nch0 = (C0 + cic - 1) / cic, nch1 = (Cin - C0 + cic - 1) / cic;
    p.nchunks = nch0 + nch1;
    p.M = M;
    p.Mp = ((M + pl.BM - 1) / pl.BM) * pl.BM;
    p.n_mtiles = p.Mp / pl.BM;
    p.act = act;
    p.epi = epi;
    p.si = si;
    p.so = so;
    p.po = po;
    p.Z = Z;
    p.C0 = C0;
    p.C1 = Cin - C0;
    const size_t per_z = (size_t)std::max(p.nchunks, 1) * p.KCp * p.Mp;
    std::vector<float> packed(per_z * Z, 0.f);
    for (int z = 0; z < Z; ++z)
        for (int m = 0; m < M; ++m)
            for (int ci = 0; ci < Cin; ++ci)
                for (int j = 0; j < taps.ntaps; ++j) {
                    const int cs = ci < C0 ? ci : ci - C0;
                    const int chunk = (ci < C0 ? 0 : nch0) + cs / cic, cil = cs % cic;
                    const size_t dst = z * per_z + ((size_t)chunk * p.KCp + (cil * taps.ntaps + j)) * p.Mp + m;
                    packed[dst] = w[(((size_t)z * M + m) * Cin + ci) * taps.ntaps + j];
                }
    p.A_z = (long)per_z;
    pl.dA = to_device(packed);
    p.A = pl.dA;
    if (M <= 4 && (epi == EPI_ACT || epi == EPI_ADD || epi == EPI_MUL || (epi == EPI_GLU && M % 2 == 0))) {
        const int MM = M <= 1 ? 1 : (M <= 2 ? 2 : 4);
        std::vector<float> ws((size_t)Z * Cin * taps.ntaps * MM, 0.f);
        for (int z = 0; z < Z; ++z)
            for (int m = 0; m < M; ++m)
                for (int ci = 0; ci < Cin; ++ci)
                    for (int j = 0; j < taps.ntaps; ++j)
                        ws[(((size_t)z * Cin + ci) * taps.ntaps + j) * MM + m] = w[(((size_t)z * M + m) * Cin + ci) * taps.ntaps + j];
        pl.dWs = to_device(ws);
        p.Ws = pl.dWs;
        pl.small.dfmin = pl.small.dfmax = taps.df[0];
        pl.small.dtmin = pl.small.dtmax = taps.dt[0];
        for (int j = 1; j < taps.ntaps; ++j) {
            pl.small.dfmin = std::min(pl.small.dfmin, taps.df[j]);
            pl.small.dfmax = std::max(pl.small.dfmax, taps.df[j]);
            pl.small.dtmin = std::min(pl.small.dtmin, taps.dt[j]);
            pl.small.dtmax = std::max(pl.small.dtmax, taps.dt[j]);
        }
    }
    if (!bias.empty()) {
        SE_CHECK((long)bias.size() == (long)Z * M, "bias size");
        pl.dBias = to_device(bias);
        p.bias = pl.dBias;
        p.bias_z = M;
    }
    if (!slope.empty()) {
        SE_CHECK((long)slope.size() == M, "slope size");
        pl.dSlope = to_device(slope);
        p.slope = pl.dSlope;
    }
    return pl;
}

static std::vector<std::pair<const char*, const char*>>& gc_safe_ranges() {
    static std::vector<std::pair<const char*, const char*>> r;
    return r;
}
static std::mutex& gc_safe_mutex() {
    static std::mutex m;
    return m;
}
void gc_register_overread_range(const void* lo, size_t bytes) {
    std::lock_guard<std::mutex> lk(gc_safe_mutex());
    gc_safe_ranges().emplace_back(static_cast<const char*>(lo), static_cast<const char*>(lo) + bytes);
}
void gc_unregister_overread_range(const void* lo) {
    std::lock_guard<std::mutex> lk(gc_safe_mutex());
    auto& r = gc_safe_ranges();
    for (size_t i = 0; i < r.size(); ++i)
        if (r[i].first == lo) {
            r.erase(r.begin() + i);
            return;
        }
}
static bool gc_overread_ok(const void* ptr) {
    if (!ptr) return true;
    std::lock_guard<std::mutex> lk(gc_safe_mutex());
    for (const auto& r : gc_safe_ranges())
        if (ptr >= r.first && static_cast<const char*>(ptr) + 16 <= r.second) return true;
    return false;
}

void gc_free_plan(GCPlan& pl) {
    if (pl.dA) (void)hipFree(pl.dA);
    if (pl.dWs) (void)hipFree(pl.dWs);
    if (pl.dDesc) (void)hipFree(pl.dDesc);
    if (pl.dDesc4) (void)hipFree(pl.dDesc4);
    pl.dDesc4 = nullptr;
    if (pl.qt2.g.tab) (void)hipFree(pl.qt2.g.tab);
    if (pl.qt2.g.desc) (void)hipFree(pl.qt2.g.desc);
    if (pl.qt2.g.desc4) (void)hipFree(pl.qt2.g.desc4);
    pl.qt2 = GCTail{};
    for (auto& t : pl.tail) {
        if (t.g.tab) (void)hipFree(t.g.tab);
        if (t.g.desc) (void)hipFree(t.g.desc);
        if (t.g.desc4) (void)hipFree(t.g.desc4);
        t = GCTail{};
    }
    for (auto& t : pl.flat) {
        if (t.g.tab) (void)hipFree(t.g.tab);
        if (t.g.desc) (void)hipFree(t.g.desc);
        if (t.g.desc4) (void)hipFree(t.g.desc4);
        t = GCTail{};
    }
    pl.dWs = nullptr;
    pl.dDesc = nullptr;
    if (pl.dBias) (void)hipFree(pl.dBias);
    if (pl.dSlope) (void)hipFree(pl.dSlope);
    if (pl.dTab) (void)hipFree(pl.dTab);
    if (pl.dBiasPad) (void)hipFree(pl.dBiasPad);
    if (pl.dPostScale) (void)hipFree(pl.dPostScale);
    if (pl.dPostShift) (void)hipFree(pl.dPostShift);
    pl.dPostScale = pl.dPostShift = nullptr;
    pl.dTab = nullptr;
    pl.dBiasPad = nullptr;
    pl.dA = pl.dBias = pl.dSlope = nullptr;
}

constexpr bool gc_flat_inst(int BM, int BN, int EPI, int UWv) {
    const bool tile = BM == 64 && (BN == 256 || BN == 128);
    if (!tile) return false;
    if (UWv == 36) return EPI == EPI_ACT || EPI == EPI_GLU || (EPI == EPI_CMB && BN == 256);
    if (UWv == 32) return EPI == EPI_ACT || (EPI == EPI_ADD && BN == 128);
    return false;
}
static bool gc_flat_supported(int BM, int BN, int epi, int uw) {
    switch (epi) {
        case EPI_ACT: return gc_flat_inst(BM, BN, EPI_ACT, uw);
        case EPI_ADD: return gc_flat_inst(BM, BN, EPI_ADD, uw);
        case EPI_GLU: return gc_flat_inst(BM, BN, EPI_GLU, uw);
        case EPI_CMB: return gc_flat_inst(BM, BN, EPI_CMB, uw);
        default: return false;
    }
}
template <int BM, int BN, int WM, int WN, int EPI, bool NRMv, int UWv>
static void gc_launch_flat_k(const GCParams& p, long nblk, size_t lds, hipStream_t stream) {
    static bool attr_fl[64] = {};
    if (first_on_device(attr_fl)) {
        SE_HIP(hipFuncSetAttribute(reinterpret_cast<const void*>(&gc_kernel<BM, BN, WM, WN, EPI, false, false, false, NRMv, UWv>),
                                   hipFuncAttributeMaxDynamicSharedMemorySize, 160 * 1024));
    }
    hipLaunchKernelGGL((gc_kernel<BM, BN, WM, WN, EPI, false, false, false, NRMv, UWv>), dim3((unsigned)nblk), dim3(256), lds, stream, p);
    SE_HIP(hipGetLastError());
    gc_log_launch(GC_FAM_TILE, p, nblk, BM, BN);
}

template <int BM, int BN, int WM, int WN, int EPI, bool RES = false>
static void gc_launch_e(const GCParams& p_in, hipStream_t stream) {
    const size_t epi = (size_t)(4 * (BM / WM) * 36) * sizeof(float);
    const size_t lds = gc_lds_bytes(p_in, BM, epi, RES ? p_in.nbuf : 2);
    static bool attr_set[64] = {};
    if (first_on_device(attr_set)) {
        SE_HIP(hipFuncSetAttribute(reinterpret_cast<const void*>(&gc_kernel<BM, BN, WM, WN, EPI, RES>),
                                   hipFuncAttributeMaxDynamicSharedMemorySize, 160 * 1024));
    }
    const long nblk = (long)p_in.Z * (p_in.flat_upr ? 1 : p_in.B) * p_in.Qt * p_in.n_ttiles * p_in.n_mtiles;
    SE_CHECK(nblk > 0 && nblk < (1L << 31), "grid size");
    const GCParams& p = p_in;
    if (p.flat_upr) {
        const int uw = p.Wp / (BN / 32);
        SE_CHECK(!RES && !p.fz && !p.trim && !p.qt2 && p.pw4 && p.t_base == 0, "gc_launch: flattened tiles on a launch they do not cover");
        const bool nrm = p.nrm0 || p.nrm1;
        if constexpr (!RES && gc_flat_inst(BM, BN, EPI, 36)) {
            if (uw == 36) {
                if constexpr (EPI == EPI_ACT && BM == 64) {
                    if (nrm) {
                        SE_CHECK(p.causal && p.Z == 1 && p.C0 + p.C1 <= GC_NRM_MAXC, "gc_launch: on-the-fly InstanceNorm needs causal taps and <= 128 input channels");
                        SE_CHECK(gc_flat_rows_spanned(p.B, p.flat_upr, BN / 32) <= GC_FLAT_NRM_ROWS,
                                 "gc_launch: a flattened tile with on-the-fly InstanceNorm would span more batch rows than it holds parameters for");
                        gc_launch_flat_k<BM, BN, WM, WN, EPI, true, 36>(p, nblk, lds, stream);
                        return;
                    }
                }
                SE_CHECK(!nrm, "gc_launch: this flattened variant cannot normalise its sources on the fly");
                gc_launch_flat_k<BM, BN, WM, WN, EPI, false, 36>(p, nblk, lds, stream);
                return;
            }
        }
        if constexpr (!RES && gc_flat_inst(BM, BN, EPI, 32)) {
            if (uw == 32) {
                if constexpr (EPI == EPI_ACT && BM == 64) {
                    if (nrm) {
                        SE_CHECK(p.causal && p.Z == 1 && p.C0 + p.C1 <= GC_NRM_MAXC, "gc_launch: on-the-fly InstanceNorm needs causal taps and <= 128 input channels");
                        SE_CHECK(gc_flat_rows_spanned(p.B, p.flat_upr, BN / 32) <= GC_FLAT_NRM_ROWS,
                                 "gc_launch: a flattened tile with on-the-fly InstanceNorm would span more batch rows than it holds parameters for");
                        gc_launch_flat_k<BM, BN, WM, WN, EPI, true, 32>(p, nblk, lds, stream);
                        return;
                    }
                }
                SE_CHECK(!nrm, "gc_launch: this flattened variant cannot normalise its sources on the fly");
                gc_launch_flat_k<BM, BN, WM, WN, EPI, false, 32>(p, nblk, lds, stream);
                return;
            }
        }
        SE_CHECK(false, "gc_launch: no flattened variant of this kernel");
    }
    if constexpr ((EPI == EPI_ACT || EPI == EPI_ADD) && !RES) {
        if (p.fz) {
            SE_CHECK(!p.trim && !p.stats, "gc_launch: no trimming / statistics variant of the kernel with the folded interaction");
            static bool attr_fz[64] = {};
            if (first_on_device(attr_fz)) {
                SE_HIP(hipFuncSetAttribute(reinterpret_cast<const void*>(&gc_kernel<BM, BN, WM, WN, EPI, false, false, true>),
                                           hipFuncAttributeMaxDynamicSharedMemorySize, 160 * 1024));
            }
            hipLaunchKernelGGL((gc_kernel<BM, BN, WM, WN, EPI, false, false, true>), dim3((unsigned)nblk), dim3(256), lds, stream, p);
            SE_HIP(hipGetLastError());
            gc_log_launch(GC_FAM_TILE, p, nblk, BM, BN);
            return;
        }
    }
    SE_CHECK(!p.fz, "gc_launch: this kernel variant cannot fold the branch interaction into its store");
    if constexpr (EPI == EPI_ACT && BM == 64 && !RES) {
        if (p.nrm0 || p.nrm1) {
            SE_CHECK(!p.trim && p.causal && !p.qt2 && p.Z == 1 && p.C0 + p.C1 <= GC_NRM_MAXC,
                     "gc_launch: on-the-fly InstanceNorm needs causal taps, one-row tiles and <= 128 input channels");
            static bool attr_nrm[64] = {};
            if (first_on_device(attr_nrm)) {
                SE_HIP(hipFuncSetAttribute(reinterpret_cast<const void*>(&gc_kernel<BM, BN, WM, WN, EPI, false, false, false, true>),
                                           hipFuncAttributeMaxDynamicSharedMemorySize, 160 * 1024));
            }
            hipLaunchKernelGGL((gc_kernel<BM, BN, WM, WN, EPI, false, false, false, true>), dim3((unsigned)nblk), dim3(256), lds, stream, p);
            SE_HIP(hipGetLastError());
            gc_log_launch(GC_FAM_TILE, p, nblk, BM, BN);
            return;
        }
    }
    SE_CHECK(!p.nrm0 && !p.nrm1, "gc_launch: this kernel variant cannot normalise its sources on the fly");
    if constexpr (EPI == EPI_ACT && !RES) {
        if (p.trim) {
            static bool attr_trim[64] = {};
            if (first_on_device(attr_trim)) {
                SE_HIP(hipFuncSetAttribute(reinterpret_cast<const void*>(&gc_kernel<BM, BN, WM, WN, EPI, false, true>),
                                           hipFuncAttributeMaxDynamicSharedMemorySize, 160 * 1024));
            }
            hipLaunchKernelGGL((gc_kernel<BM, BN, WM, WN, EPI, false, true>), dim3((unsigned)nblk), dim3(256), lds, stream, p);
            SE_HIP(hipGetLastError());
            gc_log_launch(GC_FAM_TILE, p, nblk, BM, BN);
            return;
        }
    }
    SE_CHECK(!p.trim, "gc_launch: no trimming variant of this kernel");
    hipLaunchKernelGGL((gc_kernel<BM, BN, WM, WN, EPI, RES>), dim3((unsigned)nblk), dim3(256), lds, stream, p);
    SE_HIP(hipGetLastError());
    gc_log_launch(GC_FAM_TILE, p, nblk, BM, BN, RES);
}

template <int BM, int BN, int WM, int WN, bool RES = false>
static void gc_launch_t(const GCParams& p, hipStream_t stream) {
    switch (p.epi) {
        case EPI_ACT: gc_launch_e<BM, BN, WM, WN, EPI_ACT, RES>(p, stream); break;
        case EPI_ADD: gc_launch_e<BM, BN, WM, WN, EPI_ADD, RES>(p, stream); break;
        case EPI_MUL: gc_launch_e<BM, BN, WM, WN, EPI_MUL, RES>(p, stream); break;
        case EPI_GLU: gc_launch_e<BM, BN, WM, WN, EPI_GLU, RES>(p, stream); break;
        case EPI_CMB:
            if constexpr (!RES && BM >= 64) gc_launch_e<BM, BN, WM, WN, EPI_CMB>(p, stream);
            else SE_CHECK(false, "no resident-K / 32-row form of the combine epilogue");
            break;
        case EPI_LSTM:
            if constexpr (!RES) gc_launch_e<BM, BN, WM, WN, EPI_LSTM>(p, stream);
            else SE_CHECK(false, "no resident-K form of the LSTM step");
            break;
        default: SE_CHECK(false, "unknown epilogue");
    }
}
static bool gc_resident_fits(GCParams& p, int BM, int BM_div_WM) {
    if (p.trim || p.epi == EPI_LSTM || p.epi == EPI_CMB || p.fz || p.nrm0 || p.nrm1 || p.cstats) return false;
    const long nblk = (long)p.Z * p.B * p.Q * p.n_ttiles * p.n_mtiles;
    const int nch0 = p.C0 > 0 ? (p.C0 + p.CI_C - 1) / p.CI_C : 0, nch1 = p.C1 > 0 ? (p.C1 + p.CI_C - 1) / p.CI_C : 0;
    int nb = std::max(std::max(nch0, nch1), 1);
    if (nblk > 256 || nb <= 2 || p.Tout - p.t_base > 64) return false;
    const size_t epi = (size_t)(4 * BM_div_WM * 36) * sizeof(float);
    while (nb > 2 && gc_lds_bytes(p, BM, epi, nb) > 158 * 1024) --nb;
    if (nb <= 2) return false;
    p.nbuf = nb;
    return true;
}

bool gc_nrm_supported(const GCPlan& pl) {
    static const bool on = !(getenv("SE_IN_FOLD") && atoi(getenv("SE_IN_FOLD")) == 0);
    return on && !pl.p.Ws && pl.p.epi == EPI_ACT && pl.BM == 64 && pl.p.causal && pl.p.Z == 1 && pl.p.C0 + pl.p.C1 <= GC_NRM_MAXC;
}

bool gc_stats_supported(const GCPlan& pl) {
    return !pl.p.Ws && (pl.p.epi == EPI_GLU || (pl.p.epi == EPI_ACT && pl.BM == 64));
}

void gc_launch(const GCPlan& pl, GCParams p, hipStream_t stream) {
    SE_CHECK(p.C0 == pl.p.C0 && p.C1 == pl.p.C1, "gc_launch: source channel split differs from the plan");
    SE_CHECK(!p.dst_elu || (p.epi == EPI_GLU && p.Z == 1), "gc_launch: the second (ELU) store belongs to the gated epilogue");
    if (p.epi == EPI_LSTM && p.first_step && p.C1 == 0) p.C0 = 0;
    g_flat_nrm_refused = 0;
    if (p.t_base > 0 && gc_thin_launch(p, stream)) return;
    if (p.tb_soft) p.t_base &= ~3;
    const int tb = p.t_base, Tspan = p.Tout - tb;
    SE_CHECK(tb >= 0 && (tb & 3) == 0 && Tspan > 0, "gc_launch: first output frame must be a multiple of 4 below Tout");
    SE_CHECK(tb == 0 || (!p.stats && !p.cstats), "gc_launch: the statistics epilogue needs whole rows");
    p.n_ttiles = (Tspan + pl.BN - 1) / pl.BN;
    p.Qt = p.Q;
    p.qt2 = 0;
    p.qq_off = 0;
    static const int dbg_env = getenv("SE_GC_DBG") ? atoi(getenv("SE_GC_DBG")) : 0;
    p.dbg = dbg_env;
    SE_CHECK((double)p.CI_C * (double)std::max(p.s0_c, p.s1_c) + (double)p.Fin * (double)std::max(p.s0_f, p.s1_f) + p.Tin < 1.0e9,
             "gc_launch: source plane too large for 32-bit patch byte offsets");
    constexpr long trim_min = 8192;
    const bool trim_ok = p.epi == EPI_ACT && (long)p.Z * p.B * p.Q * p.n_ttiles * p.n_mtiles >= trim_min;
    p.pw4 = (p.desc4 && (p.Tin % 4 == 0 || ((p.causal || trim_ok) && gc_overread_ok(p.src0) && gc_overread_ok(p.src1)))) ? 1 : 0;
    p.trim = (p.pw4 && !p.causal && p.Tin % 4 != 0) ? 1 : 0;
    SE_CHECK(!p.stats || gc_stats_supported(pl), "gc_launch: this tile configuration has no statistics epilogue");
    SE_CHECK(!p.cstats || (gc_stats_supported(pl) && p.n_mtiles == 1 && p.Z == 1),
             "gc_launch: column statistics need a statistics tile configuration and one m-tile (M " + std::to_string(p.M) + ", BM " +
                 std::to_string(pl.BM) + ", m-tiles " + std::to_string(p.n_mtiles) + ", epilogue " + std::to_string(p.epi) + ", direct " +
                 std::to_string(p.Ws != nullptr) + ")");
    SE_CHECK(p.pw4 || p.CI_C * p.nrows * p.Wp <= gc_bld_max(pl.BM) * 256,
             "pointwise layer with a row length that is not a multiple of 4 needs its sources inside the engine arena");
    if (gc_thin_launch(p, stream)) return;
    if (p.Ws) {
        SE_CHECK(!p.fz, "gc_launch: the direct (<= 4 channel) path cannot fold the branch interaction into its store");
        SE_CHECK(!p.dst_elu, "gc_launch: the direct (<= 4 channel) path has no second (ELU) store");
        SE_CHECK(!p.nrm0 && !p.nrm1, "gc_launch: the direct (<= 4 channel) path cannot normalise its sources on the fly");
        if (p.M <= 1) gc_small_launch<1>(p, pl.small, stream);
        else if (p.M <= 2) gc_small_launch<2>(p, pl.small, stream);
        else gc_small_launch<4>(p, pl.small, stream);
        return;
    }
    {
        const GCTail& alt = pl.tail[1];
        const long nblk = (long)p.Z * p.B * p.Q * p.n_ttiles * p.n_mtiles;
        static const int alt_n64 = getenv("SE_GC_ALT_N64") ? atoi(getenv("SE_GC_ALT_N64")) : 4096;
        if (alt.BN == 64 && nblk < (pl.BM == 64 ? alt_n64 : 256)) {
            GCParams pa = p;
            pa.n_ttiles = (Tspan + 63) / 64;
            pa.Wp = alt.Wp;
            pa.tab = alt.g.tab;
            pa.desc = alt.g.desc;
            pa.desc4 = alt.g.desc4;
            constexpr long alt32_max = 512;
            const long nblk64 = (long)p.Z * p.B * p.Q * pa.n_ttiles * p.n_mtiles;
            if (pl.BM == 128 && pl.tail[0].BN == 32 && nblk64 < alt32_max) {
                pa.n_ttiles = (Tspan + 31) / 32;
                pa.Wp = pl.tail[0].Wp;
                pa.tab = pl.tail[0].g.tab;
                pa.desc = pl.tail[0].g.desc;
                pa.desc4 = pl.tail[0].g.desc4;
                if (gc_resident_fits(pa, 128, 32)) gc_launch_t<128, 32, 4, 1, true>(pa, stream);
                else gc_launch_t<128, 32, 4, 1>(pa, stream);
                return;
            }
            if (pl.BM == 64) {
                if (gc_resident_fits(pa, 64, 32)) gc_launch_t<64, 64, 2, 2, true>(pa, stream);
                else gc_launch_t<64, 64, 2, 2>(pa, stream);
            } else {
                gc_launch_t<128, 64, 4, 1>(pa, stream);
            }
            return;
        }
    }
    {
        static const int flat_env = getenv("SE_GC_FLAT") ? atoi(getenv("SE_GC_FLAT")) : 1;
        constexpr long flat_min = 1024;
        static const long wide_min = getenv("SE_GC_WIDE_MIN") ? atol(getenv("SE_GC_WIDE_MIN")) : 6144;
        const long nblk = (long)p.Z * p.B * p.Q * p.n_ttiles * p.n_mtiles;
        const int upr = (Tspan + 31) / 32;
        const double sbmax = 4.0 * (double)std::max(p.s0_b, p.s1_b);
        if (flat_env && pl.BM == 64 && pl.flat_uw && tb == 0 && p.pw4 && !p.trim && !p.fz && p.Z == 1 && nblk >= flat_min && p.B > 1) {
            const bool wide = pl.BM == 64 && pl.flat[1].BN == 256 && nblk >= wide_min && gc_flat_supported(64, 256, p.epi, pl.flat_uw);
            const GCTail& fg = wide ? pl.flat[1] : pl.flat[0];
            const int upt = wide ? 8 : 4;
            const long tiles_plain = (long)p.B * ((Tspan + 32 * upt - 1) / (32 * upt));
            const long tiles_flat = ((long)p.B * upr + upt - 1) / upt;
            const double span = ((double)(upt + upr - 1) / upr + 1.0) * sbmax;
            const int nrm_rows = (p.nrm0 || p.nrm1) ? gc_flat_rows_spanned(p.B, upr, upt) : 0;
            const bool nrm_ok = nrm_rows <= GC_FLAT_NRM_ROWS;
            const bool flat_ok = fg.BN && gc_flat_supported(pl.BM, fg.BN, p.epi, pl.flat_uw) && tiles_flat * 100 <= tiles_plain * 94 &&
                                 span < 3.0e9;
            if (flat_ok && !nrm_ok) g_flat_nrm_refused = nrm_rows;
            if (flat_ok && nrm_ok) {
                GCParams pa = p;
                pa.flat_upr = upr;
                pa.flat_units = p.B * upr;
                pa.n_ttiles = (int)tiles_flat;
                pa.Wp = fg.Wp;
                pa.tab = fg.g.tab;
                pa.desc = fg.g.desc;
                pa.desc4 = fg.g.desc4;
                if (wide) gc_launch_t<64, 256, 1, 4>(pa, stream);
                else gc_launch_t<64, 128, 2, 2>(pa, stream);
                return;
            }
        }
    }
    {
        const GCTail& wd = pl.tail[2];
        static const long wide_min = getenv("SE_GC_WIDE_MIN") ? atol(getenv("SE_GC_WIDE_MIN")) : 6144;
        const long nblk = (long)p.Z * p.B * p.Q * p.n_ttiles * p.n_mtiles;
        const int nt = (Tspan + 255) / 256;
        static const int wide_fill = getenv("SE_GC_WIDE_FILL") ? atoi(getenv("SE_GC_WIDE_FILL")) : 75;
        if (wd.BN == 256 && pl.BM == 64 && p.pw4 && nblk >= wide_min && Tspan * 100 >= nt * 256 * wide_fill &&
            (long)p.CI_C * p.nrows * wd.Wp <= 4608 ) {
            GCParams pa = p;
            pa.n_ttiles = nt;
            pa.Wp = wd.Wp;
            pa.tab = wd.g.tab;
            pa.desc = wd.g.desc;
            pa.desc4 = wd.g.desc4;
            gc_launch_t<64, 256, 1, 4>(pa, stream);
            return;
        }
    }
    {
        const GCTail& wd = pl.tail[2];
        constexpr long wide128_min = 1536;
        constexpr int wide128_fill = 75;
        const long nblk = (long)p.Z * p.B * p.Q * p.n_ttiles * p.n_mtiles;
        const int nt = (Tspan + 255) / 256;
        if (wd.BN == 256 && pl.BM == 128 && p.epi == EPI_LSTM && p.pw4 && !p.trim && !p.stats && nblk >= wide128_min &&
            Tspan * 100L >= (long)nt * 256 * wide128_fill) {
            GCParams pa = p;
            pa.n_ttiles = nt;
            pa.Wp = wd.Wp;
            pa.tab = wd.g.tab;
            pa.desc = wd.g.desc;
            pa.desc4 = wd.g.desc4;
            gc_launch_e<128, 256, 2, 2, EPI_LSTM>(pa, stream);
            return;
        }
    }
    {
        static const long qt2_min = getenv("SE_GC_QT2_MIN") ? atol(getenv("SE_GC_QT2_MIN")) : 4096;
        const long nblk = (long)p.Z * p.B * p.Q * p.n_ttiles * p.n_mtiles;
        if (pl.qt2.BN == 64 && pl.BN == 128 && p.Q >= 2 && !p.stats && !p.cstats && p.pad_lo == 0 && p.epi != EPI_LSTM &&
            !p.nrm0 && !p.nrm1 && nblk >= qt2_min) {
            GCParams pa = p;
            pa.qt2 = 1;
            pa.qq_off = pl.qt2_qoff;
            pa.nrows = pl.qt2_nrows;
            pa.Qt = (p.Q + 1) / 2;
            pa.n_ttiles = (Tspan + 63) / 64;
            pa.Wp = pl.qt2.Wp;
            pa.tab = pl.qt2.g.tab;
            pa.desc = pl.qt2.g.desc;
            pa.desc4 = pl.qt2.g.desc4;
            if (pl.BM == 128) gc_launch_t<128, 128, 2, 2>(pa, stream);
            else if (pl.BM == 64) gc_launch_t<64, 128, 2, 2>(pa, stream);
            else gc_launch_t<32, 128, 1, 4>(pa, stream);
            return;
        }
    }
    const int full = Tspan / pl.BN, rem = Tspan - full * pl.BN;
    const GCTail* tl = nullptr;
    if (pl.tail_split && full >= 1 && rem > 0 && pl.tail[0].BN && rem <= pl.tail[0].BN) tl = &pl.tail[0];
    if (tl) {
        GCParams pt = p;
        pt.t_base = tb + full * pl.BN;
        pt.n_ttiles = 1;
        pt.Wp = tl->Wp;
        pt.tab = tl->g.tab;
        pt.desc = tl->g.desc;
        pt.desc4 = tl->g.desc4;
        p.n_ttiles = full;
        if (pl.BM == 128 && tl->BN == 32) gc_launch_t<128, 32, 4, 1>(pt, stream);
        else if (pl.BM == 128 && tl->BN == 64) gc_launch_t<128, 64, 4, 1>(pt, stream);
        else if (pl.BM == 64 && tl->BN == 64) gc_launch_t<64, 64, 2, 2>(pt, stream);
        else SE_CHECK(false, "no gemmconv tail tile config");
    }
    if (pl.BM == 128 && pl.BN == 128) gc_launch_t<128, 128, 2, 2>(p, stream);
    else if (pl.BM == 64 && pl.BN == 128) gc_launch_t<64, 128, 2, 2>(p, stream);
    else if (pl.BM == 32 && pl.BN == 128) gc_launch_t<32, 128, 1, 4>(p, stream);
    else if (pl.BM == 128 && pl.BN == 64) gc_launch_t<128, 64, 4, 1>(p, stream);
    else if (pl.BM == 64 && pl.BN == 64) gc_launch_t<64, 64, 2, 2>(p, stream);
    else SE_CHECK(false, "no gemmconv tile config");
}

}
```

Before: 2694 utt/s.

## Split conv GEMM grid into row classes that skip padded edge taps

Frequency rows near the plane edges have kernel taps that fall outside the input and were computed as zero-padded work. The change groups output rows into runs with the same set of valid taps and builds a reduced weight pack and descriptor geometry for each edge run, cached per plane. A single launch then carries up to four row classes, and each block finds its class from blockIdx and uses a smaller K. This cuts padded MACs on paired-tap BM=128 qt2 launches, at the cost of per-block class lookup, extra weight copies, an eager-only build step and a new kernel variant that may change occupancy.

```diff
diff --git a/sixty-years-of-frequency-domain-monaural-speech-enhancement_amd/csrc/gemmconv.h b/sixty-years-of-frequency-domain-monaural-speech-enhancement_amd/csrc/gemmconv.h
--- a/sixty-years-of-frequency-domain-monaural-speech-enhancement_amd/csrc/gemmconv.h
+++ b/sixty-years-of-frequency-domain-monaural-speech-enhancement_amd/csrc/gemmconv.h
@@ -23,6 +23,20 @@
 };
 
 constexpr int GC_THIN_NT = 8;
+
+constexpr int GC_MAX_CLS = 4;
+struct GCRowClass {
+    const float* A;
+    long A_z;
+    const int* tab;
+    const unsigned* desc;
+    const unsigned* desc4;
+    int CI_C, KCp, nrows, Wp;
+    int qt2, qq_off;
+    int Qt, n_ttiles;
+    int q0, q1;
+    int blk0, nblk;
+};
 
 struct GCParams {
     const float* A;
@@ -84,6 +98,8 @@
     const float* nrm1;
     int flat_upr;
     int flat_units;
+    int ncls;
+    GCRowClass cls[GC_MAX_CLS];
 };
 constexpr int GC_NRM_MAXC = 128;
 constexpr int GC_FLAT_NRM_ROWS = 2;
@@ -101,6 +117,27 @@
 struct GCSmallGeom {
     int dfmin = 0, dfmax = 0, dtmin = 0, dtmax = 0;
 };
+
+struct TapSpec {
+    int ntaps = 0;
+    int df[GC_MAX_TAPS];
+    int dt[GC_MAX_TAPS];
+};
+
+struct GCEdgeCache;
+struct GCRowRun {
+    int q0 = 0, q1 = 0;
+    std::vector<int> taps;
+};
+std::vector<GCRowRun> gc_row_runs(const TapSpec& taps, int si, int Fin, int Q);
+struct GCClassLayout {
+    int run = 0;
+    int q0 = 0, q1 = 0, qt2 = 0, Qt = 0, n_ttiles = 0;
+    long blk0 = 0, nblk = 0;
+};
+std::vector<GCClassLayout> gc_class_layout(const std::vector<GCRowRun>& runs, int ntaps, long per_tile, int ntt_two, int ntt_one);
+void gc_set_cls_min_share_pct(int pct);
+int gc_cls_min_share_pct();
 
 struct GCPlan {
     GCParams p{};
@@ -124,12 +161,7 @@
     float* dBiasPad = nullptr;
     float* dPostScale = nullptr;
     float* dPostShift = nullptr;
-};
-
-struct TapSpec {
-    int ntaps = 0;
-    int df[GC_MAX_TAPS];
-    int dt[GC_MAX_TAPS];
+    GCEdgeCache* edge = nullptr;
 };
 
 GCPlan gc_make_plan(int M, int Cin, const TapSpec& taps, const std::vector<float>& w_logical,
@@ -155,6 +187,9 @@
     int flat_nrm_refused = 0;
     long nblk = 0;
     int epi = 0, gru = 0;
+    int ncls = 0;
+    long kskip = 0;
+    long kpad = 0;
 };
 void gc_set_launch_log(std::vector<GCLaunchRec>* log);
 int gc_flat_rows_spanned(int B, int upr, int upt);
diff --git a/sixty-years-of-frequency-domain-monaural-speech-enhancement_amd/csrc/gemmconv.hip b/sixty-years-of-frequency-domain-monaural-speech-enhancement_amd/csrc/gemmconv.hip
--- a/sixty-years-of-frequency-domain-monaural-speech-enhancement_amd/csrc/gemmconv.hip
+++ b/sixty-years-of-frequency-domain-monaural-speech-enhancement_amd/csrc/gemmconv.hip
@@ -4,6 +4,7 @@
 #include <algorithm>
 #include <cmath>
 #include <cstring>
+#include <deque>
 #include <mutex>
 #include <type_traits>
 
@@ -133,7 +134,7 @@
     return x;
 }
 
-template <int BM, int BN, int WM, int WN, int EPI, bool RES = false, bool TRIM = false, bool FZ = false, bool NRM = false, int FLATW = 0>
+template <int BM, int BN, int WM, int WN, int EPI, bool RES = false, bool TRIM = false, bool FZ = false, bool NRM = false, int FLATW = 0, bool CLS = false>
 __global__ __launch_bounds__(256, RES ? 1 : (FZ || (BM >= 128 && BN >= 256)) ? (BM <= 32 ? 4 : 2) : gc_blocks_per_cu(BM)) void gc_kernel(const GCParams p) {
 #ifdef GC_TIMING
     unsigned long long tacc[12] = {0, 0, 0, 0, 0, 0, 0, 0, 0, 0, 0, 0};
@@ -145,19 +146,45 @@
     constexpr int UW = FLAT ? FLATW : 32;
     constexpr int UPT = BN / 32;
     static_assert(!FLAT || (!RES && !TRIM && !FZ && EPI != EPI_LSTM), "flattened column tiles: plain offline variants only");
+    static_assert(!CLS || (!RES && !TRIM && !FZ && !NRM && !FLAT && EPI != EPI_LSTM), "row classes: plain offline variants only");
     constexpr int KCP_MAX = gc_kcp_max(BM);
     constexpr int A_IT = (KCP_MAX * BM / 4 + 255) / 256;
     constexpr int NB = BN >= 256 ? (BM >= 128 ? 6 : 5) : gc_bld_max(BM);
     static_assert(WM * WN == 4, "4 waves");
 
     extern __shared__ __attribute__((aligned(16))) float smem[];
-    const int rows = p.CI_C * p.nrows;
-    const int npatch = rows * p.Wp;
+    int lid;
+    int c_CI_C = p.CI_C, c_nrows = p.nrows, c_Wp = p.Wp, c_KCp = p.KCp, c_Qt = p.Qt, c_ntt = p.n_ttiles, c_qt2 = p.qt2, c_qqoff = p.qq_off;
+    int c_q0 = 0, c_q1 = p.Q;
+    const float* c_A = p.A;
+    long c_Az = p.A_z;
+    const int* c_tab = p.tab;
+    const unsigned* c_desc = p.desc;
+    const unsigned* c_desc4 = p.desc4;
+    if constexpr (!CLS) {
+        const int nblk = gridDim.x, id = blockIdx.x;
+        const int xcd = id & 7, slot = id >> 3, q8 = nblk >> 3, r8 = nblk & 7;
+        lid = (xcd < r8 ? xcd * (q8 + 1) : r8 * (q8 + 1) + (xcd - r8) * q8) + slot;
+    } else {
+        const int id = blockIdx.x;
+        int ci = 0;
+#pragma unroll
+        for (int k = 1; k < GC_MAX_CLS; ++k)
+            if (k < p.ncls && id >= p.cls[k].blk0) ci = k;
+        const GCRowClass& rc = p.cls[ci];
+        c_CI_C = rc.CI_C; c_nrows = rc.nrows; c_Wp = rc.Wp; c_KCp = rc.KCp; c_Qt = rc.Qt; c_ntt = rc.n_ttiles; c_qt2 = rc.qt2; c_qqoff = rc.qq_off;
+        c_q0 = rc.q0; c_q1 = rc.q1;
+        c_A = rc.A; c_Az = rc.A_z; c_tab = rc.tab; c_desc = rc.desc; c_desc4 = rc.desc4;
+        const int s0 = rc.blk0, s1 = rc.blk0 + rc.nblk, xcd = id & 7;
+        lid = ((s1 >> 3) * xcd + min(s1 & 7, xcd)) - ((s0 >> 3) * xcd + min(s0 & 7, xcd)) + (id >> 3) - ((s0 + 7 - xcd) >> 3);
+    }
+    const int rows = c_CI_C * c_nrows;
+    const int npatch = rows * c_Wp;
     const int bit = (npatch + 255) >> 8;
     const bool pw4 = p.pw4 != 0;
     constexpr bool fixt = TRIM;
     const int bit4 = (npatch / 4 + 255) >> 8;
-    const int nA4 = p.KCp * (BM / 4);
+    const int nA4 = c_KCp * (BM / 4);
     const int ait = (nA4 + 255) >> 8;
     const int As_sz = ait * 1024;
     const int Bs_sz = bit * 256;
@@ -172,27 +199,21 @@
     const int l31 = lane & 31;
     const int hi = lane >> 5;
 
-    int lid;
-    {
-        const int nblk = gridDim.x, id = blockIdx.x;
-        const int xcd = id & 7, slot = id >> 3, q8 = nblk >> 3, r8 = nblk & 7;
-        lid = (xcd < r8 ? xcd * (q8 + 1) : r8 * (q8 + 1) + (xcd - r8) * q8) + slot;
-    }
     const int mt = lid % p.n_mtiles;
     int rest = lid / p.n_mtiles;
-    const int ttile = FLAT ? (rest / p.Qt) % p.n_ttiles : rest % p.n_ttiles;
-    if (FLAT) rest = (rest % p.Qt) + (rest / (p.Qt * p.n_ttiles)) * p.Qt;
-    else rest /= p.n_ttiles;
-    const bool qt2 = !FLAT && p.qt2 != 0;
-    const int q = (rest % p.Qt) << (qt2 ? 1 : 0);
-    rest /= p.Qt;
+    const int ttile = FLAT ? (rest / c_Qt) % c_ntt : rest % c_ntt;
+    if (FLAT) rest = (rest % c_Qt) + (rest / (c_Qt * c_ntt)) * c_Qt;
+    else rest /= c_ntt;
+    const bool qt2 = !FLAT && c_qt2 != 0;
+    const int q = c_q0 + ((rest % c_Qt) << (qt2 ? 1 : 0));
+    rest /= c_Qt;
     const int u0 = FLAT ? ttile * UPT : 0;
     const int b = FLAT ? u0 / p.flat_upr : rest % p.B;
     const int z = FLAT ? rest : rest / p.B;
     const int t0 = FLAT ? p.t_base + (u0 - b * p.flat_upr) * 32 : p.t_base + ttile * (qt2 ? BN / 2 : BN);
     const int m0 = mt * BM;
 
-    const float* __restrict__ Ag = p.A + (long)z * p.A_z + m0;
+    const float* __restrict__ Ag = c_A + (long)z * c_Az + m0;
 
     constexpr int NPAIR = KCP_MAX / 2;
     constexpr bool KOFF_REGS = (BM >= 128 || TM * TN >= 4);
@@ -208,7 +229,7 @@
     int* utab = reinterpret_cast<int*>(nrmC + (NRM ? NRMB * GC_NRM_MAXC + 2 * NRMB * KCP_MAX + 2 : 0));
     float* cpart = smem + STRIPS;
     GC_T(7);
-    const int tabv = (tid < GC_TAB_KOFF + KCP_MAX + 8) ? p.tab[tid] : 0;
+    const int tabv = (tid < GC_TAB_KOFF + KCP_MAX + 8) ? c_tab[tid] : 0;
     const int fo = q * p.so + p.po;
     const float* __restrict__ bias = (fo < p.pad_lo) ? p.bias_pad : (p.bias ? p.bias + (long)z * p.bias_z : nullptr);
     float epv[4] = {0.f, 0.f, 1.f, 0.f};
@@ -278,7 +299,7 @@
             const int f = q * p.si + tabl[tabl[GC_MAX_ROWS + kr_ - nk_cil * p.ntaps]];
             nk_ok = kr_ < p.KC && f >= 0 && f < p.Fin;
         }
-        pb_cil = tid / p.nrows;
+        pb_cil = tid / c_nrows;
     }
 
     unsigned aoff[A_IT];
@@ -305,9 +326,9 @@
     const int wq = (qt2 && WN >= 2) ? wn / WNT : 0;
     const int wt = (qt2 && WN >= 2) ? wn % WNT : wn;
     const int am = wm * (TM * 32) + l31;
-    const int bn = FLAT ? wn * (TN * UW) + l31 : wq * p.qq_off + wt * (TN * 32) + l31;
+    const int bn = FLAT ? wn * (TN * UW) + l31 : wq * c_qqoff + wt * (TN * 32) + l31;
     const int jact = FLAT ? max(0, min(TN, p.flat_units - u0 - wn * TN))
-                          : (q + wq >= p.Q) ? 0 : max(0, min(TN, (p.Tout - t0 - wt * (TN * 32) + 31) >> 5));
+                          : (q + wq >= c_q1) ? 0 : max(0, min(TN, (p.Tout - t0 - wt * (TN * 32) + 31) >> 5));
 
     int gchunk = 0;
     int buf = 0;
@@ -321,7 +342,7 @@
          \
         unsigned dsc_[NB];                                                                         \
         {                                                                                          \
-            const unsigned* __restrict__ dp_ = (pw4 ? p.desc4 : p.desc) + tid;                     \
+            const unsigned* __restrict__ dp_ = (pw4 ? c_desc4 : c_desc) + tid;                     \
             static_for<NB>([&](auto E) {                                                           \
                 constexpr int e = decltype(E)::value;                                              \
                 dsc_[e] = dp_[256 * e];                                                            \
@@ -373,7 +394,7 @@
         if constexpr (NRM) {                                                                       \
              \
              \
-            const int cb_ = (CH) * p.CI_C, co_ = seg ? p.C0 : 0;                                   \
+            const int cb_ = (CH) * c_CI_C, co_ = seg ? p.C0 : 0;                                   \
             if (tid < NRMB * KCP_MAX) {                                                            \
                 const int db_ = tid >= KCP_MAX ? 1 : 0;                                            \
                 floatx4 v_ = nrmC[db_ * GC_NRM_MAXC + min(cb_ + nk_cil, Cseg - 1) + co_];          \
@@ -385,7 +406,7 @@
             }                                                                                      \
             if (npadL > 0 && tid < rows) {                                                         \
                 const float x0_ = nrmC[min(cb_ + pb_cil, Cseg - 1) + co_][3];                      \
-                float* d_ = Bs + (BUF) * Bs_sz + tid * p.Wp;                                       \
+                float* d_ = Bs + (BUF) * Bs_sz + tid * c_Wp;                                       \
                 for (int w_ = 0; w_ < npadL; w_ += 4) *reinterpret_cast<floatx4*>(d_ + w_) = floatx4{x0_, x0_, x0_, x0_}; \
             }                                                                                      \
             if constexpr (FLAT) {       \
@@ -393,7 +414,7 @@
                     _Pragma("unroll") for (int k_ = 0; k_ < UPT; ++k_) {                           \
                         if (utab[4 * k_ + 1] + p.dtmin < 0 && utab[4 * k_ + 2]) {                  \
                             const float x0_ = nrmC[utab[4 * k_] * GC_NRM_MAXC + min(cb_ + pb_cil, Cseg - 1) + co_][3]; \
-                            float* d_ = Bs + (BUF) * Bs_sz + tid * p.Wp + k_ * UW;                 \
+                            float* d_ = Bs + (BUF) * Bs_sz + tid * c_Wp + k_ * UW;                 \
                             for (int w_ = 0; w_ < -(utab[4 * k_ + 1] + p.dtmin); w_ += 4)          \
                                 *reinterpret_cast<floatx4*>(d_ + w_) = floatx4{x0_, x0_, x0_, x0_}; \
                         }                                                                          \
@@ -403,7 +424,7 @@
         }                                                                                          \
          \
          \
-        const float* __restrict__ Bc = sbase + (long)(CH) * p.CI_C * s_c;                          \
+        const float* __restrict__ Bc = sbase + (long)(CH) * c_CI_C * s_c;                          \
         const unsigned bb = __builtin_amdgcn_readfirstlane(lds_addr(Bs + (BUF) * Bs_sz));          \
         const unsigned bl = bb + 256u * wave_u, bl4 = bb + 1024u * wave_u;                         \
         if (pw4 && fullbits == (1u << bit4) - 1u) {      \
@@ -422,7 +443,7 @@
                 if (e < bit) gc_dma4_masked_s(Bc, boff[e], bl + 1024u * e, vbits, 1u << e);         \
             });                                                                                    \
         }                                                                                          \
-        const float* __restrict__ Ac = Ag + (long)(gchunk + (CH)) * p.KCp * p.Mp;                  \
+        const float* __restrict__ Ac = Ag + (long)(gchunk + (CH)) * c_KCp * p.Mp;                  \
                                               \
         const unsigned Adw = __builtin_amdgcn_readfirstlane(lds_addr(As + (BUF) * As_sz)) + 1024u * wave_u; \
         static_for<A_IT>([&](auto I) {                                                             \
@@ -440,16 +461,16 @@
         const long s_c = seg ? p.s1_c : p.s0_c, s_f = seg ? p.s1_f : p.s0_f;
         const unsigned sc32 = (unsigned)s_c, sf32 = (unsigned)s_f;
         const unsigned sb32 = (unsigned)(seg ? p.s1_b : p.s0_b);
-        const int nch = (Cseg + p.CI_C - 1) / p.CI_C;
-        const int tail = Cseg - (nch - 1) * p.CI_C;
+        const int nch = (Cseg + c_CI_C - 1) / c_CI_C;
+        const int tail = Cseg - (nch - 1) * c_CI_C;
 
         GC_T(9);
-        GC_MAKE_DESC(nch > 1 ? p.CI_C : tail);
+        GC_MAKE_DESC(nch > 1 ? c_CI_C : tail);
         GC_T(10);
         if constexpr (RES) {
             buf = 0;
             for (int c2 = 0; c2 < min(nch, nbuf); ++c2) {
-                if (c2 + 1 == nch && nch > 1 && tail != p.CI_C) GC_MAKE_DESC(tail);
+                if (c2 + 1 == nch && nch > 1 && tail != c_CI_C) GC_MAKE_DESC(tail);
                 GC_LOAD_CHUNK(c2, c2);
             }
         } else {
@@ -467,7 +488,7 @@
                 if (c > 0 && buf == nbuf) {
                     __syncthreads();
                     for (int c2 = c; c2 < min(nch, c + nbuf); ++c2) {
-                        if (c2 + 1 == nch && tail != p.CI_C) GC_MAKE_DESC(tail);
+                        if (c2 + 1 == nch && tail != c_CI_C) GC_MAKE_DESC(tail);
                         GC_LOAD_CHUNK(c2, c2 - c);
                     }
                     GC_WAIT_CHUNK();
@@ -476,7 +497,7 @@
                 }
             }
             if (!RES && c + 1 < nch && !(p.dbg & 1)) {
-                if (__builtin_expect(c + 2 == nch && tail != p.CI_C, 0)) GC_MAKE_DESC(tail);
+                if (__builtin_expect(c + 2 == nch && tail != c_CI_C, 0)) GC_MAKE_DESC(tail);
                 GC_LOAD_CHUNK(c + 1, buf ^ 1);
             }
             GC_T(1);
@@ -488,7 +509,7 @@
 #pragma unroll
                 for (int j = 0; j < TN; ++j) nkd[j] = utab[4 * min(wn * TN + j, UPT - 1)] * KCP_MAX;
             }
-            const int npair = p.KCp >> 1;
+            const int npair = c_KCp >> 1;
 #define GC_FETCH(KP, AR, BR)                                                                       \
     {                                                                                              \
         int o_;                                                                                    \
@@ -578,7 +599,7 @@
         const int mw = wm * (TM * 32) + 4 * hi;
         const int lr = lane >> 3, lc = (lane & 7) * 4;
         const int mo0 = (EPI == EPI_GLU ? (m0 >> 1) : m0) + wm * OROWS;
-        const int Mo = (q + wq < p.Q) ? ((EPI == EPI_GLU) ? (p.M >> 1) : p.M) : 0;
+        const int Mo = (q + wq < c_q1) ? ((EPI == EPI_GLU) ? (p.M >> 1) : p.M) : 0;
         const int tvalid0 = p.tlen ? p.tlen[b] : 0x7fffffff;
         const float* __restrict__ res =
             (EPI == EPI_ADD || EPI == EPI_MUL || EPI == EPI_CMB) ? p.aux + (long)z * p.aux_z + (long)b * p.x_b + (long)fow * p.x_f : nullptr;
@@ -1278,6 +1299,7 @@
 }
 static thread_local std::vector<GCLaunchRec>* g_launch_log = nullptr;
 static thread_local int g_flat_nrm_refused = 0;
+static thread_local long g_kskip = 0, g_kpad = 0;
 void gc_set_launch_log(std::vector<GCLaunchRec>* log) { g_launch_log = log; }
 static void gc_log_launch(int family, const GCParams& p, long nblk, int BM = 0, int BN = 0, bool res = false) {
     if (!g_launch_log) return;
@@ -1298,6 +1320,9 @@
     r.nblk = nblk;
     r.epi = p.epi;
     r.gru = p.gru;
+    r.ncls = p.ncls;
+    r.kskip = p.ncls ? g_kskip : 0;
+    r.kpad = g_kpad;
     g_launch_log->push_back(r);
 }
 int gc_flat_rows_spanned(int B, int upr, int upt) {
@@ -1460,6 +1485,162 @@
     SE_HIP(hipMalloc(&g.desc4, d4.size() * sizeof(unsigned)));
     SE_HIP(hipMemcpy(g.desc4, d4.data(), d4.size() * sizeof(unsigned), hipMemcpyHostToDevice));
     return g;
+}
+
+std::vector<GCRowRun> gc_row_runs(const TapSpec& taps, int si, int Fin, int Q) {
+    std::vector<GCRowRun> runs;
+    for (int q = 0; q < Q; ++q) {
+        std::vector<int> in;
+        for (int j = 0; j < taps.ntaps; ++j) {
+            const int f = q * si + taps.df[j];
+            if (f >= 0 && f < Fin) in.push_back(j);
+        }
+        if (!runs.empty() && runs.back().taps == in) runs.back().q1 = q + 1;
+        else runs.push_back(GCRowRun{q, q + 1, in});
+    }
+    return runs;
+}
+struct GCEdgeGeom {
+    std::vector<int> taps;
+    int CI_C = 0, KCp = 0, nrows = 0;
+    GCGeom g;
+    float* dA = nullptr;
+    long A_z = 0;
+};
+struct GCEdgeSet {
+    int Fin = 0, Q = 0;
+    bool ok = false;
+    bool built = false;
+    std::vector<GCRowRun> runs;
+    std::vector<const GCEdgeGeom*> geom;
+    long pad_taps = 0;
+};
+struct GCEdgeCache {
+    TapSpec taps;
+    int si = 1, M = 0, Cin = 0, C0 = 0, Z = 1;
+    std::vector<float> w;
+    std::deque<GCEdgeGeom> geoms;
+    std::deque<GCEdgeSet> sets;
+};
+static std::mutex& gc_edge_mutex() {
+    static std::mutex m;
+    return m;
+}
+constexpr size_t GC_CLS_LDS_MAX = 48 * 1024;
+constexpr int GC_CLS_MIN_SHARE_PCT = 3;
+static int g_cls_min_share_pct = GC_CLS_MIN_SHARE_PCT;
+void gc_set_cls_min_share_pct(int pct) { g_cls_min_share_pct = pct < 0 ? GC_CLS_MIN_SHARE_PCT : pct; }
+int gc_cls_min_share_pct() { return g_cls_min_share_pct; }
+
+std::vector<GCClassLayout> gc_class_layout(const std::vector<GCRowRun>& runs, int ntaps, long per_tile, int ntt_two, int ntt_one) {
+    std::vector<int> order;
+    for (size_t i = 0; i < runs.size(); ++i) order.push_back((int)i);
+    std::stable_sort(order.begin(), order.end(), [&](int a, int b) { return runs[a].taps.size() > runs[b].taps.size(); });
+    std::vector<GCClassLayout> out;
+    long blk = 0;
+    for (int i : order) {
+        const GCRowRun& r = runs[i];
+        const int nq = r.q1 - r.q0;
+        GCClassLayout c;
+        c.run = i;
+        c.q0 = r.q0;
+        c.q1 = r.q1;
+        c.qt2 = ((int)r.taps.size() == ntaps && nq >= 2) ? 1 : 0;
+        c.Qt = c.qt2 ? (nq + 1) / 2 : nq;
+        c.n_ttiles = c.qt2 ? ntt_two : ntt_one;
+        c.blk0 = blk;
+        c.nblk = per_tile * c.Qt * c.n_ttiles;
+        blk += c.nblk;
+        out.push_back(c);
+    }
+    return out;
+}
+
+static const GCEdgeGeom* gc_edge_geom(const GCPlan& pl, GCEdgeCache& ec, const std::vector<int>& sel) {
+    for (size_t i = 0; i < ec.geoms.size(); ++i)
+        if (ec.geoms[i].taps == sel) return &ec.geoms[i];
+    const GCParams& p = pl.p;
+    TapSpec ts;
+    std::vector<int> rows;
+    for (int j : sel) {
+        ts.df[ts.ntaps] = ec.taps.df[j];
+        ts.dt[ts.ntaps] = ec.taps.dt[j];
+        ts.ntaps++;
+        if (std::find(rows.begin(), rows.end(), ec.taps.df[j]) == rows.end()) rows.push_back(ec.taps.df[j]);
+    }
+    std::sort(rows.begin(), rows.end());
+    GCEdgeGeom eg;
+    eg.taps = sel;
+    eg.nrows = (int)rows.size();
+    int cic = 0;
+    double best = -1.0;
+    for (int c = 1; c <= std::max(std::max(ec.C0, ec.Cin - ec.C0), 1); ++c) {
+        const int kc = c * ts.ntaps, kcp = (kc + 3) & ~3;
+        if (kcp > gc_kcp_max(pl.BM) || c * eg.nrows * p.Wp > gc_bld_max(pl.BM) * 256) continue;
+        GCParams t = p;
+        t.KCp = kcp;
+        t.CI_C = c;
+        t.nrows = eg.nrows;
+        if (gc_lds_bytes(t, pl.BM, (size_t)(4 * 64 * 36) * sizeof(float), 2) > GC_CLS_LDS_MAX) continue;
+        const double score = (double)kc / kcp + 1e-4 * kc;
+        if (score > best) {
+            best = score;
+            cic = c;
+        }
+    }
+    if (cic == 0) return nullptr;
+    eg.CI_C = cic;
+    const int KC = cic * ts.ntaps;
+    eg.KCp = (KC + 3) & ~3;
+    eg.g = gc_build_geom(ts, rows, p.dtmin, eg.nrows, p.Wp, cic, KC, gc_bld_max(pl.BM));
+    const int nch0 = (ec.C0 + cic - 1) / cic, nch1 = (ec.Cin - ec.C0 + cic - 1) / cic;
+    const size_t per_z = (size_t)std::max(nch0 + nch1, 1) * eg.KCp * p.Mp;
+    std::vector<float> packed(per_z * ec.Z, 0.f);
+    for (int z = 0; z < ec.Z; ++z)
+        for (int m = 0; m < ec.M; ++m)
+            for (int ci = 0; ci < ec.Cin; ++ci)
+                for (int j = 0; j < ts.ntaps; ++j) {
+                    const int cs = ci < ec.C0 ? ci : ci - ec.C0;
+                    const int chunk = (ci < ec.C0 ? 0 : nch0) + cs / cic, cil = cs % cic;
+                    packed[z * per_z + ((size_t)chunk * eg.KCp + (cil * ts.ntaps + j)) * p.Mp + m] =
+                        ec.w[(((size_t)z * ec.M + m) * ec.Cin + ci) * ec.taps.ntaps + sel[j]];
+                }
+    eg.A_z = (long)per_z;
+    eg.dA = to_device(packed);
+    ec.geoms.push_back(eg);
+    return &ec.geoms.back();
+}
+static const GCEdgeSet* gc_edge_set(const GCPlan& pl, int Fin, int Q, int min_pct, hipStream_t stream) {
+    GCEdgeCache& ec = *pl.edge;
+    std::lock_guard<std::mutex> lk(gc_edge_mutex());
+    GCEdgeSet* s = nullptr;
+    for (GCEdgeSet& c : ec.sets)
+        if (c.Fin == Fin && c.Q == Q) s = &c;
+    if (!s) {
+        GCEdgeSet n;
+        n.Fin = Fin;
+        n.Q = Q;
+        n.runs = gc_row_runs(ec.taps, ec.si, Fin, Q);
+        n.ok = (int)n.runs.size() <= GC_MAX_CLS && n.runs.size() >= 2;
+        for (const GCRowRun& r : n.runs) {
+            n.pad_taps += (long)(r.q1 - r.q0) * (ec.taps.ntaps - (int)r.taps.size());
+            if (r.taps.size() < 2) n.ok = false;
+        }
+        ec.sets.push_back(n);
+        s = &ec.sets.back();
+    }
+    if (s->ok && !s->built && s->pad_taps * 100 >= (long)Q * ec.taps.ntaps * min_pct) {
+        hipStreamCaptureStatus cap = hipStreamCaptureStatusNone;
+        SE_CHECK(hipStreamIsCapturing(stream, &cap) == hipSuccess && cap == hipStreamCaptureStatusNone,
+                 "gc_launch: the row classes of a plane must be built by an eager launch, not inside a stream capture");
+        for (const GCRowRun& r : s->runs) {
+            const GCEdgeGeom* g = (int)r.taps.size() == ec.taps.ntaps ? nullptr : gc_edge_geom(pl, ec, r.taps);
+            if (!g && (int)r.taps.size() != ec.taps.ntaps) s->ok = false;
+            s->geom.push_back(g);
+        }
+        s->built = s->ok;
+    }
+    return s;
 }
 
 GCPlan gc_make_plan(int M, int Cin, const TapSpec& taps, const std::vector<float>& w, const std::vector<float>& bias,
@@ -1610,6 +1791,20 @@
     p.A_z = (long)per_z;
     pl.dA = to_device(packed);
     p.A = pl.dA;
+    {
+        bool paired = taps.ntaps % 2 == 0 && taps.ntaps >= 4;
+        for (int j = 0; paired && j < taps.ntaps; j += 2) paired = taps.df[j] == taps.df[j + 1];
+        if (paired && pl.BM == 128 && pl.BN == 128 && pl.qt2.BN == 64 && epi == EPI_ACT) {
+            pl.edge = new GCEdgeCache;
+            pl.edge->taps = taps;
+            pl.edge->si = si;
+            pl.edge->M = M;
+            pl.edge->Cin = Cin;
+            pl.edge->C0 = C0;
+            pl.edge->Z = Z;
+            pl.edge->w = w;
+        }
+    }
     if (M <= 4 && (epi == EPI_ACT || epi == EPI_ADD || epi == EPI_MUL || (epi == EPI_GLU && M % 2 == 0))) {
         const int MM = M <= 1 ? 1 : (M <= 2 ? 2 : 4);
         std::vector<float> ws((size_t)Z * Cin * taps.ntaps * MM, 0.f);
@@ -1673,6 +1868,16 @@
 }
 
 void gc_free_plan(GCPlan& pl) {
+    if (pl.edge) {
+        for (GCEdgeGeom& eg : pl.edge->geoms) {
+            if (eg.dA) (void)hipFree(eg.dA);
+            if (eg.g.tab) (void)hipFree(eg.g.tab);
+            if (eg.g.desc) (void)hipFree(eg.g.desc);
+            if (eg.g.desc4) (void)hipFree(eg.g.desc4);
+        }
+        delete pl.edge;
+        pl.edge = nullptr;
+    }
     if (pl.dA) (void)hipFree(pl.dA);
     if (pl.dWs) (void)hipFree(pl.dWs);
     if (pl.dDesc) (void)hipFree(pl.dDesc);
@@ -1739,7 +1944,36 @@
 template <int BM, int BN, int WM, int WN, int EPI, bool RES = false>
 static void gc_launch_e(const GCParams& p_in, hipStream_t stream) {
     const size_t epi = (size_t)(4 * (BM / WM) * 36) * sizeof(float);
-    const size_t lds = gc_lds_bytes(p_in, BM, epi, RES ? p_in.nbuf : 2);
+    size_t lds = gc_lds_bytes(p_in, BM, epi, RES ? p_in.nbuf : 2);
+    if constexpr (BM == 128 && BN == 128 && WM == 2 && !RES && (EPI == EPI_ACT || EPI == EPI_CMB)) {
+        if (p_in.ncls) {
+            SE_CHECK(!p_in.flat_upr && !p_in.fz && !p_in.trim && !p_in.nrm0 && !p_in.nrm1 && !p_in.stats && !p_in.cstats,
+                     "gc_launch: row classes on a launch they do not cover");
+            long nb = 0;
+            for (int k = 0; k < p_in.ncls; ++k) {
+                const GCRowClass& rc = p_in.cls[k];
+                GCParams t = p_in;
+                t.KCp = rc.KCp;
+                t.CI_C = rc.CI_C;
+                t.nrows = rc.nrows;
+                t.Wp = rc.Wp;
+                lds = k ? std::max(lds, gc_lds_bytes(t, BM, epi, 2)) : gc_lds_bytes(t, BM, epi, 2);
+                SE_CHECK(rc.blk0 == nb && rc.nblk > 0, "gc_launch: row classes must tile the grid");
+                nb += rc.nblk;
+            }
+            SE_CHECK(nb < (1L << 31), "grid size");
+            static bool attr_cls[64] = {};
+            if (first_on_device(attr_cls)) {
+                SE_HIP(hipFuncSetAttribute(reinterpret_cast<const void*>(&gc_kernel<BM, BN, WM, WN, EPI, false, false, false, false, 0, true>),
+                                           hipFuncAttributeMaxDynamicSharedMemorySize, 160 * 1024));
+            }
+            hipLaunchKernelGGL((gc_kernel<BM, BN, WM, WN, EPI, false, false, false, false, 0, true>), dim3((unsigned)nb), dim3(256), lds, stream, p_in);
+            SE_HIP(hipGetLastError());
+            gc_log_launch(GC_FAM_TILE, p_in, nb, BM, BN);
+            return;
+        }
+    }
+    SE_CHECK(!p_in.ncls, "gc_launch: no row-class variant of this kernel");
     static bool attr_set[64] = {};
     if (first_on_device(attr_set)) {
         SE_HIP(hipFuncSetAttribute(reinterpret_cast<const void*>(&gc_kernel<BM, BN, WM, WN, EPI, RES>),
@@ -1881,6 +2115,8 @@
     SE_CHECK(!p.dst_elu || (p.epi == EPI_GLU && p.Z == 1), "gc_launch: the second (ELU) store belongs to the gated epilogue");
     if (p.epi == EPI_LSTM && p.first_step && p.C1 == 0) p.C0 = 0;
     g_flat_nrm_refused = 0;
+    g_kskip = g_kpad = 0;
+    p.ncls = 0;
     if (p.t_base > 0 && gc_thin_launch(p, stream)) return;
     if (p.tb_soft) p.t_base &= ~3;
     const int tb = p.t_base, Tspan = p.Tout - tb;
@@ -2032,6 +2268,31 @@
             pa.tab = pl.qt2.g.tab;
             pa.desc = pl.qt2.g.desc;
             pa.desc4 = pl.qt2.g.desc4;
+            const GCEdgeSet* es = nullptr;
+            if (pl.edge && pl.BM == 128 && (p.epi == EPI_ACT || p.epi == EPI_CMB) && !p.trim && !p.fz && p.A_z == pl.p.A_z &&
+                pl.p.A_z > 0 && (p.A - pl.p.A) % pl.p.A_z == 0)
+                es = gc_edge_set(pl, p.Fin, p.Q, g_cls_min_share_pct, stream);
+            if (es && es->ok) g_kpad = es->pad_taps * (p.C0 + p.C1);
+            if (es && es->built && es->pad_taps * 100 >= (long)p.Q * pl.edge->taps.ntaps * g_cls_min_share_pct) {
+                const long zoff = (p.A - pl.p.A) / pl.p.A_z;
+                for (const GCClassLayout& c : gc_class_layout(es->runs, pl.edge->taps.ntaps, (long)p.Z * p.B * p.n_mtiles, pa.n_ttiles, p.n_ttiles)) {
+                    const GCEdgeGeom* eg = es->geom[c.run];
+                    GCRowClass& rc = pa.cls[pa.ncls++];
+                    rc.q0 = c.q0; rc.q1 = c.q1; rc.qt2 = c.qt2; rc.Qt = c.Qt; rc.n_ttiles = c.n_ttiles;
+                    rc.blk0 = (int)c.blk0; rc.nblk = (int)c.nblk;
+                    if (eg) {
+                        rc.A = eg->dA + zoff * eg->A_z; rc.A_z = eg->A_z; rc.tab = eg->g.tab; rc.desc = eg->g.desc; rc.desc4 = eg->g.desc4;
+                        rc.CI_C = eg->CI_C; rc.KCp = eg->KCp; rc.nrows = eg->nrows; rc.Wp = p.Wp; rc.qq_off = 0;
+                        g_kskip += (long)(c.q1 - c.q0) * (pl.edge->taps.ntaps - (long)eg->taps.size()) * (p.C0 + p.C1);
+                    } else if (c.qt2) {
+                        rc.A = p.A; rc.A_z = p.A_z; rc.tab = pa.tab; rc.desc = pa.desc; rc.desc4 = pa.desc4;
+                        rc.CI_C = p.CI_C; rc.KCp = p.KCp; rc.nrows = pa.nrows; rc.Wp = pa.Wp; rc.qq_off = pa.qq_off;
+                    } else {
+                        rc.A = p.A; rc.A_z = p.A_z; rc.tab = p.tab; rc.desc = p.desc; rc.desc4 = p.desc4;
+                        rc.CI_C = p.CI_C; rc.KCp = p.KCp; rc.nrows = p.nrows; rc.Wp = p.Wp; rc.qq_off = 0;
+                    }
+                }
+            }
             if (pl.BM == 128) gc_launch_t<128, 128, 2, 2>(pa, stream);
             else if (pl.BM == 64) gc_launch_t<64, 128, 2, 2>(pa, stream);
             else gc_launch_t<32, 128, 1, 4>(pa, stream);
```

After: 2752 utt/s (median of 6 runs). 1.02x the previous value.
